# baldhat/yolov10-3D

Measured on AMD Instinct MI355X. Metric: train_images_per_sec, higher is better.
Workload: dtype bf16

## Files before the change

include/y3d.h:

```cpp
#ifndef Y3D_H
#define Y3D_H
#include <stdint.h>

#ifdef __cplusplus
extern "C" {
#endif

enum { Y3D_F32 = 0, Y3D_BF16 = 1 };
enum { Y3D_OK = 0, Y3D_ERR_INVALID = -1, Y3D_ERR_HIP = -2 };

const char* y3d_last_error(void);
int y3d_abi_version(void);
int y3d_device_info(char* name, int name_len, int* compute_units, int* lds_bytes, int* clock_khz);

int y3d_pack_weight_fwd(int dtype, const float* w_oihw, void* out, int Cout, int Cin_g, int Cin_g_pad, int kh, int kw, void* stream);
int y3d_pack_weight_dgrad(int dtype, const float* w_oihw, void* out, int Cout, int Cin_g, int groups, int kh, int kw, void* stream);
int y3d_mt_pack_weights(int dtype, const int64_t* desc, const int* chunk_tensor, const int* chunk_off, int nchunks, int chunk, void* stream);
int y3d_mt_fp8w_quantize(const int64_t* desc, const int* row_begin, int ntensors, int nrows, void* stream);
int y3d_fp8w_dequantize(const uint8_t* codes, const float* scale, float* w, int rows, int K, void* stream);
int y3d_fp8_quantize_act(const void* x, int64_t xsw, int64_t M, int C, uint8_t* q, uint8_t* s, void* stream);
int y3d_fp8_pack_weight_fwd(const uint8_t* codes, const float* scale, int rows, int Cg, uint8_t* wq, uint8_t* ws, void* stream);
int y3d_conv3x3_fp8_ok(int B, int H, int W, int Cin, int Cout, int groups);
int y3d_conv3x3_fp8_stat_rows(int B, int H, int W);
int y3d_fp8_scale_pitch(int C);
int y3d_conv3x3_fp8_fwd(const uint8_t* xq, const uint8_t* xs, int B, int H, int W, int Cin, const uint8_t* wq, const uint8_t* ws, void* y, int64_t ysw,
                        int Cout, int groups, float* stat_partials, const float* scale, const float* shift, int act, void* stream);
int y3d_fp8_quantize_grad(const void* dy, int64_t sw, const float* scale, int64_t M, int C, uint8_t* q, uint8_t* s, void* stream);
int y3d_fp8_pack_weight_dgrad(const uint8_t* codes, int Cout, int Cin, int groups, int lo, int hi, uint8_t* wq, uint8_t* ws, void* stream);
int y3d_conv3x3_fp8_dgrad_ok(int B, int H, int W, int Cin, int Cout, int groups);
int y3d_conv3x3_fp8_dgrad(const uint8_t* dyq, const uint8_t* dys, int64_t qsw, int spitch, int lo, int hi, int B, int H, int W, const uint8_t* wq, const uint8_t* ws,
                          void* dx, int64_t dxsw, int Cin, int groups, void* stream);
int y3d_conv_kpad(int dtype, int k_total);
int y3d_conv_stat_blocks(int B, int Ho, int Wo);
int y3d_conv2d_stat_rows(int dtype, int B, int H, int W, int Cin, int Cout, int groups, int kh, int kw, int stride, int pad);
enum { Y3D_OP_FWD = 0, Y3D_OP_BWD_DATA = 1, Y3D_OP_BWD_WEIGHT = 2 };
enum { Y3D_EPI_RAW = 0, Y3D_EPI_PARTIALS = 1, Y3D_EPI_AFFINE = 2, Y3D_EPI_AFFINE_RES = 3, Y3D_EPI_BIAS = 4 };
enum {
  Y3D_ROUTE_GENERIC = 0,
  Y3D_ROUTE_STREAM1X1 = 1,
  Y3D_ROUTE_SMALL = 2,
  Y3D_ROUTE_SMALL_S2 = 3,
  Y3D_ROUTE_S2_DGRAD = 4,
  Y3D_ROUTE_TILE8 = 5,
  Y3D_ROUTE_TILE16 = 6,
  Y3D_ROUTE_WIDE3_8 = 7,
  Y3D_ROUTE_WIDE3_16 = 8,
  Y3D_ROUTE_FLAT = 9,
  Y3D_ROUTE_WGRAD_SMALL = 10,
  Y3D_ROUTE_WGRAD_TILE = 11,
  Y3D_ROUTE_WGRAD_STREAM1X1 = 12
};
int y3d_conv2d_route(int dtype, int op, int epi, int B, int H, int W, int Cin, int Cout, int groups, int kh, int kw, int stride, int pad);
int y3d_conv2d_fwd(int dtype, const void* x, int64_t xsb, int64_t xsh, int64_t xsw, int B, int H, int W, int Cin,
                   const void* w_packed, const float* bias, void* y, int64_t ysw, int Ho, int Wo, int Cout, int groups,
                   int kh, int kw, int stride, int pad, float* stat_partials, void* stream);
int y3d_conv2d_fwd_affine(int dtype, const void* x, int64_t xsb, int64_t xsh, int64_t xsw, int B, int H, int W, int Cin,
                          const void* w_packed, const float* scale, const float* shift, int act, void* y, int64_t ysw, int Ho, int Wo,
                          int Cout, int groups, int kh, int kw, int stride, int pad, void* stream);
int y3d_conv2d_fwd_affine_res_ok(int dtype, int B, int H, int W, int Cin, int Cout, int groups, int kh, int kw, int stride, int pad);
int y3d_conv2d_fwd_affine_res(int dtype, const void* x, int64_t xsb, int64_t xsh, int64_t xsw, int B, int H, int W, int Cin,
                              const void* w_packed, const float* scale, const float* shift, int act, const void* res, int64_t rsw, void* y,
                              int64_t ysw, int Ho, int Wo, int Cout, int groups, int kh, int kw, int stride, int pad, void* stream);
int y3d_conv2d_bwd_data(int dtype, const void* dy, int64_t dsb, int64_t dsh, int64_t dsw, int B, int Ho, int Wo, int Cout,
                        const void* w_packed_dgrad, void* dx, int64_t xsw, int H, int W, int Cin, int groups, int kh, int kw,
                        int stride, int pad, void* stream);
int y3d_conv2d_wgrad_splits(int dtype, int B, int Ho, int Wo, int Cout, int Cin_g, int groups, int kh, int kw);
int y3d_conv2d_wgrad_plan(int dtype, int B, int H, int W, int Cin, int Cout, int groups, int kh, int kw, int stride, int pad);
int y3d_set_tile_kernels(int enable);
int y3d_set_stream1x1(int enable);
int y3d_get_stream1x1(void);
int y3d_get_tile_kernels(void);
int y3d_set_bn_wide_slabs(int enable);
int y3d_conv2d_bwd_weight(int dtype, const void* x, int64_t xsb, int64_t xsh, int64_t xsw, int B, int H, int W, int Cin,
                          int Cin_real, const void* dy, int64_t dsw, int Ho, int Wo, int Cout, int groups, int kh, int kw,
                          int stride, int pad, float* slab, int nsplit, float* grad_oihw, int accumulate, void* stream);

int y3d_dw_blocks(int64_t M);
int y3d_dw_wgrad_blocks(int64_t M);
int y3d_dw_pack_weight(const float* w_oihw, float* out_taps_c, int C, int kh, int kw, void* stream);
int y3d_dwconv2d_fwd(int dtype, const void* x, int64_t xsb, int64_t xsh, int64_t xsw, int B, int H, int W, int C,
                     const float* w_packed, void* y, int64_t ysw, int Ho, int Wo, int kh, int kw, int stride, int pad,
                     float* stat_partials, void* stream);
int y3d_dwconv2d_fwd_affine(int dtype, const void* x, int64_t xsb, int64_t xsh, int64_t xsw, int B, int H, int W, int C,
                            const float* w_packed, const float* scale, const float* shift, int act, int res_mode, const void* res, int64_t rsw,
                            void* z, int64_t zsw, int Ho, int Wo, int kh, int kw, int stride, int pad, void* stream);
int y3d_dwconv2d_bwd_data(int dtype, const void* dy, int64_t dsb, int64_t dsh, int64_t dsw, int B, int Ho, int Wo, int C,
                          const float* w_packed, void* dx, int64_t xsw, int H, int W, int kh, int kw, int stride, int pad,
                          void* stream);
int y3d_dwconv2d_bwd_weight(int dtype, const void* x, int64_t xsb, int64_t xsh, int64_t xsw, int B, int H, int W, int C,
                            const void* dy, int64_t dsw, int Ho, int Wo, int kh, int kw, int stride, int pad, float* slab,
                            float* grad_oihw, int accumulate, void* stream);

int y3d_bn_finalize(const float* partials, int nblk, int C, int64_t count, const float* gamma, const float* beta, float eps,
                    float momentum, float* running_mean, float* running_var, float* mean, float* invstd, float* scale,
                    float* shift, void* stream);
int y3d_bn_eval_scale(int C, const float* gamma, const float* beta, const float* running_mean, const float* running_var,
                      float eps, float* scale, float* shift, void* stream);
int y3d_bn_act_fwd(int dtype, const void* y, int64_t ysw, const float* scale, const float* shift, int act, int res_mode,
                   const void* res, int64_t rsw, void* z, int64_t zsw, int64_t P, int C, void* stream);
int y3d_bn_act_fwd_q(const void* y, int64_t ysw, const float* scale, const float* shift, int act, void* z, int64_t zsw, uint8_t* q, uint8_t* s,
                     int64_t P, int C, void* stream);
int y3d_bn_bwd_blocks(int64_t P, int C);
int y3d_bn_act_bwd_reduce(int dtype, const void* y, int64_t ysw, const void* dz, int64_t dsw, const void* res, int64_t rsw,
                          const float* scale, const float* shift, const float* mean, const float* invstd, int act,
                          int res_mode, float* partials, int64_t P, int C, void* stream);
int y3d_bn_bwd_finalize(const float* partials, int nblk, int C, int64_t count, float* dgamma, float* dbeta, int accumulate,
                        float* mean_g, float* mean_gx, void* stream);
int y3d_bn_act_bwd_apply(int dtype, const void* y, int64_t ysw, const void* dz, int64_t dsw, const void* res, int64_t rsw,
                         const float* scale, const float* shift, const float* mean, const float* invstd,
                         const float* mean_g, const float* mean_gx, int act, int res_mode, int train, void* dy, int64_t dysw,
                         void* dres, int64_t drsw, int64_t P, int C, void* stream);
int y3d_colsum_partials(int dtype, const void* x, int64_t xsw, float* partials, int64_t P, int C, void* stream);

int y3d_maxpool_fwd(int dtype, const void* x, int64_t xsb, int64_t xsh, int64_t xsw, void* y, int64_t ysw, uint8_t* argmax,
                    int B, int H, int W, int C, int k, void* stream);
int y3d_maxpool_bwd(int dtype, const void* dy, int64_t dsw, const uint8_t* argmax, void* dx, int64_t xsw, int B, int H, int W,
                    int C, int k, void* stream);
int y3d_upsample2x_fwd(int dtype, const void* x, int64_t xsb, int64_t xsh, int64_t xsw, void* y, int64_t ysw, int B, int H, int W,
                       int C, void* stream);
int y3d_upsample2x_bwd(int dtype, const void* dy, int64_t dsb, int64_t dsh, int64_t dsw, void* dx, int64_t xsw, int B, int H,
                       int W, int C, void* stream);
int y3d_copy2d(int dtype, const void* x, int64_t xsw, void* y, int64_t ysw, int64_t P, int C, void* stream);
int y3d_occupy_cus(int n, const int* flag, float* buf, int64_t nbuf, void* stream);
int y3d_add2d(int dtype, const void* a, int64_t asw, const void* b, int64_t bsw, void* y, int64_t ysw, int64_t P, int C, void* stream);
int y3d_nchw_to_nhwc(int dtype, const float* x_nchw, void* y_nhwc, int B, int C, int H, int W, int Cpad, void* stream);
int y3d_stem_im2col(int dtype, const float* x_nchw, void* out, int B, int H, int W, int Ho, int Wo, void* stream);
int y3d_stem_im2col_u8(int dtype, const uint8_t* x, int hwc, void* out, int B, int H, int W, int Ho, int Wo, void* stream);
int y3d_stem_conv_eval(const void* x, int in_mode, const float* wcol, const float* scale, const float* shift, int act, void* y, int64_t ysw,
                       int B, int H, int W, int Cout, void* stream);
int y3d_stem_conv_train_rows(int B, int H, int W);
int y3d_stem_conv_train(const void* x, int in_mode, const float* wcol, void* y, int64_t ysw, void* xcol, float* part, int B, int H, int W,
                        int Cout, void* stream);
int y3d_nhwc_to_nchw(int dtype, const void* x_nhwc, int64_t xsw, float* y_nchw, int B, int C, int H, int W, void* stream);
int y3d_proj_fwd(int dtype, const void* x, int64_t xsw, const float* w, const float* bias, void* y, int64_t ysw, int64_t P,
                 int Cin, int Cout, void* stream);
int y3d_proj_bwd_data(int dtype, const void* dy, int64_t dsw, const float* w, void* dx, int64_t xsw, int64_t P, int Cin, int Cout,
                      void* stream);
int y3d_proj_blocks(int64_t P);
int y3d_proj_bwd_weight(int dtype, const void* x, int64_t xsw, const void* dy, int64_t dsw, float* slab, float* bias_slab,
                        float* grad_w, float* grad_b, int accumulate, int64_t P, int Cin, int Cout, void* stream);
int y3d_slab_reduce(const float* slab, float* out, int nblk, int64_t n, int accumulate, void* stream);
int y3d_proj_group_fwd(int dtype, int nb, int cin, const void* x, int64_t xsw, const int* xoff, const float* const* w,
                       const float* const* b, const int* couts, void* y, int64_t ysw, int64_t P, void* stream);
int y3d_proj_group_bwd_data(int dtype, int nb, int cin, const void* dy, int64_t dsw, const int* xoff, const float* const* w,
                            const int* couts, void* dx, int64_t xsw, int64_t P, void* stream);
int y3d_proj_group_fwd_bn_mfma(int nb, int cin, const void* y_pre, int64_t ysw, const int* xoff, const float* const* w, const float* const* b,
                               const int* couts, const float* scale, const float* shift, int act, void* out, int64_t osw, int64_t P,
                               void* stream);
int y3d_proj_group_bwd_weight_bn_mfma_blocks(int64_t P);
int y3d_proj_group_bwd_weight_bn_mfma(int nb, int cin, const void* y_pre, int64_t ysw, const int* xoff, const void* dout, int64_t dsw,
                                      const int* couts, const float* scale, const float* shift, int act, float* slab, float* bslab,
                                      float* const* dw, float* const* db, int64_t P, void* stream);
int y3d_proj_group_bn_bwd_blocks(int64_t P);
int y3d_proj_group_bn_bwd(int mode, int nb, int cin, const void* y_pre, int64_t ysw, const int* xoff, const void* dout, int64_t dsw,
                          const float* const* w, const int* couts, const float* scale, const float* shift, const float* mean,
                          const float* invstd, const float* mean_g, const float* mean_gx, int act, float* partials, int nblk, void* dy,
                          int64_t dysw, int64_t P, int C, void* stream);
int y3d_proj_group_blocks(int64_t P);
int y3d_proj_group_fwd_bn(int dtype, int nb, int cin, const void* y_pre, int64_t xsw, const int* xoff, const float* const* w,
                          const float* const* b, const int* couts, const float* scale, const float* shift, int act, void* out,
                          int64_t ysw, int64_t P, void* stream);
int y3d_proj_group_bwd_weight_bn(int dtype, int nb, int cin, const void* y_pre, int64_t xsw, const int* xoff, const void* dy, int64_t dsw,
                                 const int* couts, const float* scale, const float* shift, int act, float* slab, float* bslab,
                                 float* const* dw, float* const* db, int64_t P, void* stream);
int y3d_proj_group_bwd_weight(int dtype, int nb, int cin, const void* x, int64_t xsw, const int* xoff, const void* dy, int64_t dsw,
                              const int* couts, float* slab, float* bslab, float* const* dw, float* const* db, int64_t P, void* stream);

int y3d_attn_fwd(int dtype, const void* qkv, int64_t qsw, void* out, int64_t osw, float* lse, int B, int N, int nh, int kd, int hd,
                 float scale, void* stream);
int y3d_attn_bwd(int dtype, const void* qkv, int64_t qsw, const void* out, int64_t osw, const void* dout, int64_t dsw,
                 const void* dv_extra, int64_t esw, const float* lse, float* delta, void* dqkv, int64_t gsw, int B, int N, int nh,
                 int kd, int hd, float scale, void* stream);

int y3d_tal3d_scratch_floats(int B, int n, int A, int topk);
int y3d_pad_targets(const float* rows, int nbox, int width, int B, int cap, float scale_x, float scale_y, float* out, int* n_used,
                    void* stream);
int y3d_tal3d_assign(int dtype, int nl, const void* const* maps, const int64_t* psw, const int* H, const int* W, const float* strides,
                     int B, int nc, const float* gt, int n, const float* calib, const float* mean_sizes, int topk, float alpha,
                     float beta, float gamma, int mode, float* scratch, uint8_t* fg_mask, int* target_gt_idx, float* target_scores, float* scal,
                     const int* n_used, void* stream);
int y3d_loss3d(int dtype, int nl, const void* const* maps, const int64_t* psw, void* const* grads, const int64_t* gsw, const int* H,
               const int* W, const float* strides, int B, int nc, const float* gt, int n, const uint8_t* fg_mask,
               const int* target_gt_idx, const float* target_scores, const float* scal, float w_loss2d, float w_cls, float w_depth,
               float w_offset3d, float w_size3d, float w_heading, float grad_scale, float* partials, float* items, void* stream);

int y3d_distill_loss(int dtype, int nl, const void* const* embs, const int64_t* psw, const int* H, const int* W, int B, int C,
                     const void* teacher, int teacher_dtype, int th, int tw, int64_t tsb, int64_t tsc, int64_t tsh, int64_t tsw,
                     const float* gt, int n, const uint8_t* fg_mask, const int* target_gt_idx, const float* scal, const uint8_t* mixed,
                     int img_w, int img_h, float T, float weight, int criterion, int no_mixup, int cap, int* counts, int* idx,
                     void* rows, float* partials, float* loss, void* stream);
int y3d_distill_scatter(int dtype, const void* rows, const int* idx, const int* nrows, const float* scale, int cap, int C, void* grad,
                        int64_t sb, int64_t sh, int64_t sw, int a0, int H, int W, void* stream);

int y3d_tal2d_assign(int dtype, int nl, const void* const* maps, const int64_t* psw, const int* H, const int* W, const float* strides,
                     int B, int nc, const float* gt, int n, int topk, float alpha, float beta, float* scratch, uint8_t* fg_mask,
                     int* target_gt_idx, float* target_scores, float* scal, const int* n_used, void* stream);
int y3d_loss2d(int dtype, int nl, const void* const* maps, const int64_t* psw, void* const* grads, const int64_t* gsw, const int* H,
               const int* W, const float* strides, int B, int nc, const float* gt, int n, const uint8_t* fg_mask,
               const int* target_gt_idx, const float* target_scores, const float* scal, float w_box, float w_cls, float w_dfl,
               float grad_scale, float* partials, float* items, void* stream);
int y3d_tal2d_scratch_floats(int B, int n, int A, int topk);
int y3d_tal2d_assign_crowded(int dtype, int nl, const void* const* maps, const int64_t* psw, const int* H, const int* W, const float* strides,
                             int B, int nc, const float* gt, int n, int topk, float alpha, float beta, float* scratch, uint8_t* fg_mask,
                             int* target_gt_idx, float* target_scores, float* scal, const int* n_used, void* stream);

int y3d_topk_cells(int dtype, const void* cls, int64_t psw, int B, int HW, int nc, int K, int* out_idx, void* stream);
int y3d_patch_gather(int dtype, const void* x, int64_t xsb, int64_t xsh, int64_t xsw, const int* idx, void* out, int B, int H, int W,
                     int C, int K, int ps, void* stream);
int y3d_head3d_scatter(int dtype, const void* cls, int64_t csw, const void* reg, int64_t rsw, const int* idx, void* map, int B, int HW,
                       int nc, int no, int K, void* stream);
int y3d_head3d_decode(int dtype, int nl, const void* const* maps, const int* H, const int* W, const float* strides, int B, int nc,
                      float* y, void* stream);
int y3d_head2d_decode(int dtype, int nl, const void* const* maps, const int* H, const int* W, const float* strides, int B, int nc,
                      float* y, void* stream);
int y3d_v10_postprocess_scratch_floats(int B, int A, int nc, int max_det);
int y3d_v10_postprocess(const float* y, int B, int C, int A, int nc, int max_det, int boxes_first, float* reg, float* scores,
                        int64_t* labels, float* scratch, void* stream);

int y3d_kitti_image_aug(const unsigned char* const* src, const unsigned char* const* src2, const int* hw, const int* flip, const double* trans_inv,
                        int B, int out_h, int out_w, int mode, void* out, void* stream);
int y3d_kde_depth_fusion(const float* predsO, int B, int K, const float* predsM, int KM, int C, float thres, float iou_thres, int nprop,
                         float* out, void* stream);
int y3d_kitti_decode(const float* preds, int B, int K, const double* calib, const double* ratio, const double* inv_trans,
                     const double* mean_size, int nc, int use_camera_dis, double threshold, double* out, unsigned char* keep, void* stream);
int y3d_kitti_encode_labels(const double* rec, const int* img_i, const double* img_f, int B, int out_w, int out_h, double min_depth,
                            double max_depth, int use_camera_dis, const double* mean_size, int n_cls, int max_objs, int64_t* cls,
                            double* bboxes, float* center_2d, float* size_2d, double* center_3d, double* size_3d, double* depth,
                            int64_t* heading_bin, double* heading_res, float* batch_idx, int* counts, double* calib, double* ratio_pad,
                            void* stream);
int y3d_kitti_plan_batch(const int64_t* img_off, const int* frame_hw, const int* rec_span, const float* P2, int N,
                         const unsigned char* arena, const double* draws_host, const double* draws, int B, const unsigned char** src,
                         const unsigned char** src2, int* hw, int* flip, double* trans_inv, int* img_i, double* img_f,
                         unsigned char* mixed, void* stream);
int y3d_json3d_encode_labels(const double* rec, const int* img_i, const double* img_f, int B, int dataset, int out_w, int out_h,
                             double min_depth, double max_depth, int use_camera_dis, const double* mean_size, int n_cls, int max_objs,
                             int64_t* cls, double* bboxes, float* center_2d, float* size_2d, double* center_3d, double* size_3d,
                             double* depth, int64_t* heading_bin, double* heading_res, float* batch_idx, int* counts, double* calib,
                             double* ratio_pad, void* stream);
int y3d_yolo2d_image_aug(const unsigned char* const* src, int n_src, const int* rec_i, const double* rec_f, const unsigned char* lut, int B,
                         int imgsz, int mode, void* out, void* stream);
int y3d_yolo2d_encode_labels(const float* rec, int n_rec, const int* lab_i, const float* lab_f, int B, int imgsz, int cap, float* cls,
                             float* bboxes, float* batch_idx, int* counts, void* stream);
int y3d_letterbox_image(const unsigned char* const* src_table, int n_src, const int* rec, int B, int H, int W, int mode, void* out,
                        void* stream);
// ... 55 lines not shown
```

yolov10-3d_amd/csrc/common.h:

```cpp
#pragma once
#include <hip/hip_runtime.h>
#include <stdint.h>

#include "../../include/y3d.h"

typedef unsigned short bf16_t;
typedef __attribute__((ext_vector_type(8))) __bf16 bf16x8_t;
typedef __attribute__((ext_vector_type(4))) float f32x4_t;
typedef __attribute__((ext_vector_type(4))) short s16x4_t;

#define Y3D_WAVE 64

__device__ __forceinline__ float bf2f(bf16_t v) { return __uint_as_float(((unsigned)v) << 16); }
__device__ __forceinline__ bf16_t f2bf(float f) {
  __bf16 b = (__bf16)f;
  return __builtin_bit_cast(unsigned short, b);
}

template <typename T> struct TT;
template <> struct TT<float> {
  static constexpr int CE = 4;
  static constexpr int BKE = 32;
  __device__ static __forceinline__ float ld(const float* p) { return *p; }
  __device__ static __forceinline__ void st(float* p, float v) { *p = v; }
  __device__ static __forceinline__ float rnd(float v) { return v; }
};
template <> struct TT<bf16_t> {
  static constexpr int CE = 8;
  static constexpr int BKE = 64;
  __device__ static __forceinline__ float ld(const bf16_t* p) { return bf2f(*p); }
  __device__ static __forceinline__ void st(bf16_t* p, float v) { *p = f2bf(v); }
  __device__ static __forceinline__ float rnd(float v) { return bf2f(f2bf(v)); }
};

template <typename T> struct Chunk;
template <> struct Chunk<float> {
  __device__ static __forceinline__ void unpack(const uint4& u, float* f) {
    f[0] = __uint_as_float(u.x); f[1] = __uint_as_float(u.y); f[2] = __uint_as_float(u.z); f[3] = __uint_as_float(u.w);
  }
  __device__ static __forceinline__ uint4 pack(const float* f) {
    return make_uint4(__float_as_uint(f[0]), __float_as_uint(f[1]), __float_as_uint(f[2]), __float_as_uint(f[3]));
  }
};
template <> struct Chunk<bf16_t> {
  __device__ static __forceinline__ void unpack(const uint4& u, float* f) {
    f[0] = __uint_as_float(u.x << 16); f[1] = __uint_as_float(u.x & 0xffff0000u);
    f[2] = __uint_as_float(u.y << 16); f[3] = __uint_as_float(u.y & 0xffff0000u);
    f[4] = __uint_as_float(u.z << 16); f[5] = __uint_as_float(u.z & 0xffff0000u);
    f[6] = __uint_as_float(u.w << 16); f[7] = __uint_as_float(u.w & 0xffff0000u);
  }
  __device__ static __forceinline__ uint4 pack(const float* f) {
    uint4 u;
    u.x = (unsigned)f2bf(f[0]) | ((unsigned)f2bf(f[1]) << 16);
    u.y = (unsigned)f2bf(f[2]) | ((unsigned)f2bf(f[3]) << 16);
    u.z = (unsigned)f2bf(f[4]) | ((unsigned)f2bf(f[5]) << 16);
    u.w = (unsigned)f2bf(f[6]) | ((unsigned)f2bf(f[7]) << 16);
    return u;
  }
};

__device__ __forceinline__ float fast_sigmoid_f(float u) { return __builtin_amdgcn_rcpf(1.f + __expf(-u)); }
__device__ __forceinline__ float silu_f(float u) { return u * fast_sigmoid_f(u); }
__device__ __forceinline__ float silu_grad_f(float u) {
  float s = fast_sigmoid_f(u);
  return s * (1.f + u * (1.f - s));
}

__device__ __forceinline__ float lane_xor8_sum(float v) {
  return v + __int_as_float(__builtin_amdgcn_update_dpp(0, __float_as_int(v), 0x128, 0xf, 0xf, false));
}
__device__ __forceinline__ float lane_xor16_sum(float v) {
  auto r = __builtin_amdgcn_permlane16_swap(__float_as_uint(v), __float_as_uint(v), false, false);
  return __uint_as_float(r[0]) + __uint_as_float(r[1]);
}
__device__ __forceinline__ float lane_xor32_sum(float v) {
  auto r = __builtin_amdgcn_permlane32_swap(__float_as_uint(v), __float_as_uint(v), false, false);
  return __uint_as_float(r[0]) + __uint_as_float(r[1]);
}

__device__ __forceinline__ float wave_xor_sum16(float v) {
  v += __int_as_float(__builtin_amdgcn_update_dpp(0, __float_as_int(v), 0xB1, 0xf, 0xf, false));
  v += __int_as_float(__builtin_amdgcn_update_dpp(0, __float_as_int(v), 0x4E, 0xf, 0xf, false));
  v += __int_as_float(__builtin_amdgcn_update_dpp(0, __float_as_int(v), 0x141, 0xf, 0xf, false));
  v += __int_as_float(__builtin_amdgcn_update_dpp(0, __float_as_int(v), 0x140, 0xf, 0xf, false));
  return v;
}

void y3d_set_error(const char* fmt, ...);
#define Y3D_CHECK(cond, ...)          \
  do {                                \
    if (!(cond)) {                    \
      y3d_set_error(__VA_ARGS__);     \
      return Y3D_ERR_INVALID;         \
    }                                 \
  } while (0)
#define Y3D_LAUNCH_CHECK()                                   \
  do {                                                       \
    hipError_t e_ = hipGetLastError();                       \
    if (e_ != hipSuccess) {                                  \
      y3d_set_error("HIP launch: %s", hipGetErrorString(e_)); \
      return Y3D_ERR_HIP;                                    \
    }                                                        \
  } while (0)

#define Y3D_HIP(call)                                                 \
  do {                                                                \
    hipError_t e_ = (call);                                           \
    if (e_ != hipSuccess) {                                           \
      y3d_set_error("%s: %s", #call, hipGetErrorString(e_));          \
      return Y3D_ERR_HIP;                                             \
    }                                                                 \
  } while (0)

static inline int cdiv(long a, long b) { return (int)((a + b - 1) / b); }
```

yolov10-3d_amd/csrc/conv_gemm.hip:

```cpp
#include "common.h"
#include "conv_frag.h"
#include <cstdlib>

namespace {

struct ConvP {
  const void* x;
  const void* w;
  const float* bias;
  const float* scale;
  const float* shift;
  int act;
  void* y;
  float* part;
  long xsb, xsh, xsw;
  long ysw;
  int B, Hg, Wg;
  int Hq, Wq;
  int Cg, Cn, G;
  int kh, kw, stride, pad;
  int Ktot, Kpad;
  int M;
  int ntx, nty;
};
// ... 329 lines not shown
  const T* __restrict__ X = (const T*)p.x;
  const T* __restrict__ D = (const T*)p.dy;

  const int mbeg = split * p.chunk_px;
  const int mend = min(p.M, mbeg + p.chunk_px);
  const int nsteps = (mend - mbeg + BPK - 1) / BPK;

  const int ccd = tid % CPD, rd0 = tid / CPD;
  const int ccx = tid % CPX, rx0 = tid / CPX;
  constexpr int RSD = 256 / CPD, RSX = 256 / CPX;
  const bool tdv = BPK * CPD >= 256 || tid < BPK * CPD, txv = BPK * CPX >= 256 || tid < BPK * CPX;
  const int kx = j0 + ccx * CE;
  const bool kx_ok = txv && kx < p.Ktot;
  int tap = 0, ci = 0, tr = 0, tq = 0;
  if (kx_ok) { tap = kx / p.Cg; ci = kx - tap * p.Cg; tr = tap / p.kw; tq = tap - tr * p.kw; }
  const int cd = i0 + ccd * CE;
  const bool cd_ok = tdv && cd < p.Cn;
  const int HW = p.Ho * p.Wo;

  uint4 rd[ND], rx[NX];
  int rb_[NX], rh_[NX], rw_[NX];
#pragma unroll
  for (int i = 0; i < NX; ++i) {
    int m = mbeg + rx0 + RSX * i;
    int b = m / HW;
    int rem = m - b * HW;
    rb_[i] = b;
    rh_[i] = rem / p.Wo;
    rw_[i] = rem - rh_[i] * p.Wo;
  }
  const T* dcol = D + (long)g * p.Cn + cd;
  const T* xcol = X + (long)g * p.Cg + ci + (long)(tr - p.pad) * p.xsh + (long)(tq - p.pad) * p.xsw;
  auto gload = [&](int st) {
#pragma unroll
    for (int i = 0; i < ND; ++i) {
      int m = mbeg + st * BPK + rd0 + RSD * i;
      uint4 vd = make_uint4(0, 0, 0, 0);
      if (m < mend && cd_ok) vd = *(const uint4*)(dcol + (long)m * p.dsw);
      rd[i] = vd;
    }
#pragma unroll
    for (int i = 0; i < NX; ++i) {
      int m = mbeg + st * BPK + rx0 + RSX * i;
      uint4 vx = make_uint4(0, 0, 0, 0);
      if (m < mend && kx_ok) {
        int hh = rh_[i] * p.stride - p.pad + tr, ww = rw_[i] * p.stride - p.pad + tq;
        if (hh >= 0 && ww >= 0 && hh < p.H && ww < p.W)
          vx = *(const uint4*)(xcol + (long)rb_[i] * p.xsb + (long)(rh_[i] * p.stride) * p.xsh + (long)(rw_[i] * p.stride) * p.xsw);
      }
      rx[i] = vx;
      rw_[i] += BPK;
      while (rw_[i] >= p.Wo) { rw_[i] -= p.Wo; ++rh_[i]; }
      while (rh_[i] >= p.Ho) { rh_[i] -= p.Ho; ++rb_[i]; }
    }
  };
  auto lstore = [&](int buf) {
    if (tdv) {
#pragma unroll
      for (int i = 0; i < ND; ++i) *(uint4*)(sD + buf * BPK * PD + (rd0 + RSD * i) * PD + ccd * 16) = rd[i];
    }
    if (txv) {
#pragma unroll
      for (int i = 0; i < NX; ++i) *(uint4*)(sX + buf * BPK * PX + (rx0 + RSX * i) * PX + ccx * 16) = rx[i];
    }
  };

  f32x4_t acc[TA][TB];
#pragma unroll
  for (int a = 0; a < TA; ++a)
#pragma unroll
    for (int b = 0; b < TB; ++b) acc[a][b] = (f32x4_t){0.f, 0.f, 0.f, 0.f};

  if (nsteps > 0) {
    gload(0);
    lstore(0);
  }
  __syncthreads();
  for (int st = 0; st < nsteps; ++st) {
    const int cur = st & 1;
    if (st + 1 < nsteps) gload(st + 1);
    const char* tD = sD + cur * BPK * PD;
    const char* tX = sX + cur * BPK * PX;
#pragma unroll
    for (int k0 = 0; k0 < BPK; k0 += TFrag<T, WD>::KSUB_PX) {
      typename TFrag<T, WD>::type fa[TA], fb[TB];
#pragma unroll
      for (int a = 0; a < TA; ++a) fa[a] = TFrag<T, WD>::load(tD, wi * (WD / 2) + a * 16, k0, lane);
#pragma unroll
      for (int b = 0; b < TB; ++b) fb[b] = TFrag<T, WX>::load(tX, wj * (WX / 2) + b * 16, k0, lane);
#pragma unroll
      for (int a = 0; a < TA; ++a)
#pragma unroll
        for (int b = 0; b < TB; ++b) acc[a][b] = TFrag<T, WD>::mma(fa[a], fb[b], acc[a][b]);
    }
    if (st + 1 < nsteps) lstore(cur ^ 1);
    __syncthreads();
  }
  float* slab = p.slab + ((long)split * p.G * p.Cn + (long)g * p.Cn) * p.Ktot;
#pragma unroll
  for (int a = 0; a < TA; ++a)
#pragma unroll
    for (int b = 0; b < TB; ++b) {
      int k = j0 + wj * (WX / 2) + b * 16 + (lane & 15);
#pragma unroll
      for (int r = 0; r < 4; ++r) {
        int co = i0 + wi * (WD / 2) + a * 16 + (lane >> 4) * 4 + r;
        if (co < p.Cn && k < p.Ktot) slab[(long)co * p.Ktot + k] = acc[a][b][r];
      }
    }
}

template <int SL>
__global__ __launch_bounds__(256) void wgrad_reduce_kernel(const float* __restrict__ slab, float* __restrict__ grad, int nsplit, int Ctot,
                                                           int taps, int Cg, int Cg_real, int accumulate) {
  constexpr int GPB = 256 / SL;
  __shared__ float4 sh[SL][GPB];
  const int e = threadIdx.x % GPB, sl = threadIdx.x / GPB;
  const long idx = ((long)blockIdx.x * GPB + e) * 4;
  const long n = (long)Ctot * taps * Cg;
  float4 s = make_float4(0.f, 0.f, 0.f, 0.f);
  if (idx < n) {
    float4 s0 = s, s1 = s, s2 = s, s3 = s;
    auto add = [](float4& a, const float4 b) { a.x += b.x; a.y += b.y; a.z += b.z; a.w += b.w; };
    int k = sl;
    for (; k + 3 * SL < nsplit; k += 4 * SL) {
      const float4 v0 = *(const float4*)(slab + (long)k * n + idx), v1 = *(const float4*)(slab + (long)(k + SL) * n + idx);
      const float4 v2 = *(const float4*)(slab + (long)(k + 2 * SL) * n + idx), v3 = *(const float4*)(slab + (long)(k + 3 * SL) * n + idx);
      add(s0, v0); add(s1, v1); add(s2, v2); add(s3, v3);
    }
    for (; k < nsplit; k += SL) add(s0, *(const float4*)(slab + (long)k * n + idx));
    s.x = (s0.x + s1.x) + (s2.x + s3.x); s.y = (s0.y + s1.y) + (s2.y + s3.y);
    s.z = (s0.z + s1.z) + (s2.z + s3.z); s.w = (s0.w + s1.w) + (s2.w + s3.w);
  }
  if (SL > 1) {
    sh[sl][e] = s;
    __syncthreads();
    if (sl != 0) return;
#pragma unroll
    for (int j = 1; j < SL; ++j) { const float4 v = sh[j][e]; s.x += v.x; s.y += v.y; s.z += v.z; s.w += v.w; }
  }
  if (idx >= n) return;
  const int ci = (int)(idx % Cg);
  const int tap = (int)((idx / Cg) % taps);
  const int co = (int)(idx / ((long)Cg * taps));
  const float v[4] = {s.x, s.y, s.z, s.w};
#pragma unroll
  for (int j = 0; j < 4; ++j) {
    if (ci + j >= Cg_real) break;
    const long o = ((long)co * Cg_real + ci + j) * taps + tap;
    grad[o] = accumulate ? grad[o] + v[j] : v[j];
  }
}

template <int SL>
__global__ __launch_bounds__(256) void wgrad_reduce_scalar_kernel(const float* __restrict__ slab, float* __restrict__ grad, int nsplit, int Ctot,
                                                           int taps, int Cg, int Cg_real, int accumulate) {
  constexpr int EPB = 256 / SL;
  __shared__ float sh[SL][EPB];
  const int e = threadIdx.x % EPB, sl = threadIdx.x / EPB;
  long idx = (long)blockIdx.x * EPB + e;
  long n = (long)Ctot * taps * Cg;
  float s = 0.f;
  if (idx < n) {
    float s0 = 0.f, s1 = 0.f, s2 = 0.f, s3 = 0.f;
    int k = sl;
    for (; k + 3 * SL < nsplit; k += 4 * SL) {
      s0 += slab[(long)k * n + idx];
      s1 += slab[(long)(k + SL) * n + idx];
      s2 += slab[(long)(k + 2 * SL) * n + idx];
      s3 += slab[(long)(k + 3 * SL) * n + idx];
    }
    for (; k < nsplit; k += SL) s0 += slab[(long)k * n + idx];
    s = (s0 + s1) + (s2 + s3);
  }
  if (SL > 1) {
    sh[sl][e] = s;
    __syncthreads();
    if (sl != 0) return;
#pragma unroll
    for (int j = 1; j < SL; ++j) s += sh[j][e];
  }
  if (idx >= n) return;
  int ci = idx % Cg;
  int tap = (idx / Cg) % taps;
  int co = idx / ((long)Cg * taps);
  if (ci >= Cg_real) return;
  long o = ((long)co * Cg_real + ci) * taps + tap;
  grad[o] = accumulate ? grad[o] + s : s;
}

inline void launch_wgrad_reduce(const float* slab, float* grad, int nsplit, int Ctot, int taps, int Cg, int Cg_real, int accumulate, hipStream_t st) {
  long n = (long)Ctot * taps * Cg;
  long ng = (n + 3) / 4;
  if (n <= 65536 && nsplit >= 64) hipLaunchKernelGGL(wgrad_reduce_kernel<16>, dim3(cdiv(ng, 16)), dim3(256), 0, st, slab, grad, nsplit, Ctot, taps, Cg, Cg_real, accumulate);
  else if (n <= 1048576 && nsplit >= 32) hipLaunchKernelGGL(wgrad_reduce_kernel<8>, dim3(cdiv(ng, 32)), dim3(256), 0, st, slab, grad, nsplit, Ctot, taps, Cg, Cg_real, accumulate);
  else if (nsplit >= 8) hipLaunchKernelGGL(wgrad_reduce_kernel<2>, dim3(cdiv(ng, 128)), dim3(256), 0, st, slab, grad, nsplit, Ctot, taps, Cg, Cg_real, accumulate);
  else hipLaunchKernelGGL(wgrad_reduce_scalar_kernel<1>, dim3(cdiv(n, 256)), dim3(256), 0, st, slab, grad, nsplit, Ctot, taps, Cg, Cg_real, accumulate);
}

template <typename T>
__global__ void pack_w_fwd_kernel(const float* __restrict__ w, T* __restrict__ out, int Cout, int Cg, int Cg_pad, int taps, int Kpad) {
  long idx = (long)blockIdx.x * blockDim.x + threadIdx.x;
  long n = (long)Cout * Kpad;
  if (idx >= n) return;
  int k = idx % Kpad;
  int co = idx / Kpad;
  float v = 0.f;
  if (k < taps * Cg_pad) {
    int tap = k / Cg_pad, ci = k - tap * Cg_pad;
    if (ci < Cg) v = w[((long)co * Cg + ci) * taps + tap];
  }
  TT<T>::st(out + idx, v);
}

template <typename T>
__global__ void pack_w_dgrad_kernel(const float* __restrict__ w, T* __restrict__ out, int G, int Cn, int Cg, int taps, int Kpad) {
  long idx = (long)blockIdx.x * blockDim.x + threadIdx.x;
  long n = (long)G * Cg * Kpad;
  if (idx >= n) return;
  int k = idx % Kpad;
  int ci = (idx / Kpad) % Cg;
  int g = idx / ((long)Kpad * Cg);
  float v = 0.f;
  if (k < taps * Cn) {
    int tap = k / Cn, co = k - tap * Cn;
    v = w[((long)(g * Cn + co) * Cg + ci) * taps + tap];
  }
  TT<T>::st(out + idx, v);
}

template <typename T>
__global__ __launch_bounds__(256) void mt_pack_w_kernel(const long* __restrict__ desc, const int* __restrict__ ctensor, const int* __restrict__ coff,
                                                        int chunk) {
  constexpr int CAP = 4096;
  __shared__ float st[CAP + 64];
  const long* d = desc + (long)ctensor[blockIdx.x] * 8;
  const float* __restrict__ w = (const float*)d[0];
  T* __restrict__ out = (T*)d[1];
  const int a = (int)d[2], b = (int)d[3], c = (int)d[4], taps = (int)d[5], Kpad = (int)d[6], mode = (int)d[7];
  const long n = mode == 0 ? (long)a * Kpad : (long)a * c * Kpad;
  const long beg = (long)coff[blockIdx.x] * chunk;
  const long end = beg + chunk < n ? beg + chunk : n;
  const int tid = threadIdx.x;
  const long rb = beg / Kpad, re = (end - 1) / Kpad;
  if (mode == 0) {
    for (long idx = beg + tid; idx < end; idx += 256) {
      const int k = (int)(idx % Kpad), co = (int)(idx / Kpad);
      float v = 0.f;
      if (k < taps * c) {
        const int tap = k / c, ci = k - tap * c;
        if (ci < b) v = w[((long)co * b + ci) * taps + tap];
      }
      TT<T>::st(out + idx, v);
    }
  } else {
    const int CB = b < 256 ? b : 256;
    int R = CAP / (taps * (CB + 1));
    if (R < 1) R = 1;
    const int P = CB + 1;
    for (long r0 = rb; r0 <= re;) {
      const int g = (int)(r0 / c), ci0 = (int)(r0 - (long)g * c);
      int nr = R;
      if (nr > c - ci0) nr = c - ci0;
      if (nr > re - r0 + 1) nr = (int)(re - r0 + 1);
      const int seg = nr * taps;
      for (int co0 = 0; co0 < b; co0 += CB) {
        const int cb = b - co0 < CB ? b - co0 : CB;
        __syncthreads();
        for (int i = tid; i < cb * seg; i += 256) {
          const int col = i / seg, j = i - col * seg;
          st[j * P + col] = w[((long)(g * b + co0 + col) * c + ci0) * taps + j];
        }
        __syncthreads();
        for (int o = tid; o < seg * cb; o += 256) {
          const int j = o / cb, col = o - j * cb;
          const int cil = j / taps, tap = j - cil * taps;
          const long idx = (r0 + cil) * Kpad + (long)tap * b + co0 + col;
          if (idx >= beg && idx < end) TT<T>::st(out + idx, st[j * P + col]);
        }
      }
      for (int o = tid; o < nr * (Kpad - taps * b); o += 256) {
        const int rl = o / (Kpad - taps * b), k = taps * b + o - rl * (Kpad - taps * b);
        const long idx = (r0 + rl) * Kpad + k;
        if (idx >= beg && idx < end) TT<T>::st(out + idx, 0.f);
      }
      r0 += nr;
    }
  }
}

template <typename T, int MODE>
int launch_conv_mode(ConvP p, hipStream_t st) {
  dim3 block(256);
  const unsigned ny = MODE == 2 ? 4 : 1;
  p.ntx = MODE == 2 ? cdiv((long)p.B * ((p.Hq + 1) / 2) * ((p.Wq + 1) / 2), 128) : cdiv(p.M, 128);
  const long t128 = (long)p.ntx * cdiv(p.Cn, 128) * ny * p.G;
  int bc = p.Cn > 64 ? 128 : (p.Cn > 32 ? 64 : 32);
  if (p.Cn % 32 == 0) {
    if (bc == 128 && t128 < 192) bc = 64;
    if (bc == 64 && (long)p.ntx * cdiv(p.Cn, 64) * ny * p.G < 192 && p.Cn > 32) bc = 32;
  }
  p.nty = cdiv(p.Cn, bc);
  if (bc == 128) {
    size_t sm = 2 * (128 + 128) * 128;
    hipLaunchKernelGGL((conv_gemm_kernel<T, 128, 128, 2, 2, MODE>), dim3(p.ntx * p.nty, ny, p.G), block, sm, st, p);
  } else if (bc == 64) {
    size_t sm = 2 * (128 + 64) * 128;
    hipLaunchKernelGGL((conv_gemm_kernel<T, 128, 64, 4, 1, MODE>), dim3(p.ntx * p.nty, ny, p.G), block, sm, st, p);
  } else {
    size_t sm = 2 * (128 + 32) * 128;
    hipLaunchKernelGGL((conv_gemm_kernel<T, 128, 32, 4, 1, MODE>), dim3(p.ntx * p.nty, ny, p.G), block, sm, st, p);
  }
  Y3D_LAUNCH_CHECK();
  return Y3D_OK;
}

template <typename T, bool DGRAD>
int launch_conv(ConvP p, hipStream_t st) {
  if (DGRAD && p.kh == 3 && p.kw == 3 && p.stride == 2 && p.pad == 1 && p.Cg % TT<T>::CE == 0) return launch_conv_mode<T, 2>(p, st);
  return launch_conv_mode<T, DGRAD ? 1 : 0>(p, st);
}

}

int y3d_conv3x3_tile_route(int dtype, int B, int H, int W, int Cg, int Cn, int G, int kh, int kw, int stride, int pad);
int y3d_conv3x3_flat_tiles(int B, int H, int W);
int y3d_conv3x3_tile_launch(int dtype, int route, const void* x, long xsb, long xsh, long xsw, int B, int H, int W, int Cg, int Cn, int G,
                            const void* w, int Ktot, void* y, long ysw, float* part, int flip, const float* scale, const float* shift, int act,
                            void* stream);

int y3d_wgrad_tile_height(int dtype, int H, int W, int Cg, int Cn, int kh, int kw, int stride, int pad);
int y3d_wgrad_tile_splits(int th, int B, int H, int W, int Cg, int Cn, int G);
int y3d_conv3x3_wgrad_tile_launch(int th, const void* x, long xsb, long xsh, long xsw, const void* dy, long dsw, int B, int H, int W, int Cg,
                                  int Cn, int G, float* slab, int nsplit, void* stream);

int y3d_conv1x1_stream_ok(int dtype, long M, int K, int N, long xsw, int G = 1);
int y3d_conv1x1_stream_launch(const void* x, long xsw, const void* w, int Kpad, const float* bias, const float* scale, const float* shift, int act,
                              void* y, long ysw, float* part, long M, int K, int N, int G, void* stream);
int y3d_wgrad1x1_stream_ok(int dtype, long M, int Cg, int Cn, long xsw, long dsw);
int y3d_wgrad1x1_stream_launch(const void* x, long xsw, const void* dy, long dsw, long M, int Cg, int Cn, float* slab, int nsplit, int chunk_px,
                               void* stream);
int y3d_conv3x3s2_dgrad_ok(int dtype, int B, int Ho, int Wo, int H, int W, int Cout, int Cin, long dsw, long xsw);
int y3d_conv3x3s2_dgrad_launch(const void* dy, long dsw, int B, int Ho, int Wo, int Cout, const void* w_packed_dgrad, int Kpad, void* dx, long xsw,
                               int H, int W, int Cin, void* stream);
int y3d_conv3x3_small_ok(int dtype, int B, int H, int W, int Cin, int Cout, int rows);
int y3d_conv3x3_small_launch(const void* x, long xsb, long xsh, long xsw, int B, int H, int W, int Cin, int Cout, const void* w, int Ktot, void* y,
                             long ysw, float* part, int rows, int flip, const float* scale, const float* shift, int act, const void* res, long rsw,
                             void* stream);
int y3d_conv3x3_small_rows(int B, int H, int W, int Cin, int Cout);
int y3d_conv3x3_small_s2_ok(int dtype, int B, int H, int W, int Cin, int Cout);
int y3d_conv3x3_small_s2_rows(int B, int H, int W, int Cin, int Cout);
int y3d_conv3x3_small_s2_launch(const void* x, long xsb, long xsh, long xsw, int B, int H, int W, int Cin, int Cout, const void* w, int Ktot, void* y,
                                long ysw, float* part, int rows, const float* scale, const float* shift, int act, void* stream);
int y3d_conv1x1_stream_rows(long M, int K, int N, int G = 1);
int y3d_wgrad3x3_small_ok(int dtype, int B, int H, int W, int Cin, int Cout);
int y3d_wgrad3x3_small_splits(int B, int H, int W);
int y3d_wgrad3x3_small_launch(const void* x, long xsb, long xsh, long xsw, const void* dy, long dsw, int B, int H, int W, int Cin, int Cout,
                              float* slab, int nsplit, void* stream);
static inline bool dense_pixels(int B, int H, int W, long sb, long sh, long sw) {
  return (H == 1 || sh == (long)W * sw) && (B == 1 || sb == (long)H * W * sw);
}

static int g_tile_kernels = 1;
extern "C" int y3d_conv2d_wgrad_splits(int dtype, int B, int Ho, int Wo, int Cout, int Cin_g, int groups, int kh, int kw);

static int conv_route(int dtype, int op, int epi, int B, int H, int W, int Ho, int Wo, int Cin, int Cout, int groups, int kh, int kw, int stride,
                      int pad, bool dense, long asw, long bsw, bool cin_full) {
  const int ce = dtype == Y3D_BF16 ? 8 : 4;
  const bool k1 = kh == 1 && kw == 1 && stride == 1 && pad == 0, k3s1 = kh == 3 && kw == 3 && stride == 1 && pad == 1,
             k3s2 = kh == 3 && kw == 3 && stride == 2 && pad == 1;
  if (op == Y3D_OP_FWD) {
    Y3D_CHECK(dtype == Y3D_BF16 || dtype == Y3D_F32, "conv2d_fwd: bad dtype %d", dtype);
    Y3D_CHECK(B > 0 && H > 0 && W > 0 && Cin > 0 && Cout > 0 && groups > 0, "conv2d_fwd: empty shape");
    Y3D_CHECK(Cin % groups == 0 && Cout % groups == 0, "conv2d_fwd: channels not divisible by groups");
    Y3D_CHECK((Cin / groups) % ce == 0, "conv2d_fwd: Cin/groups=%d must be a multiple of %d (pad the input)", Cin / groups, ce);
    Y3D_CHECK(kh * kw <= 64, "conv2d_fwd: at most 64 filter taps");
    Y3D_CHECK(epi >= Y3D_EPI_RAW && epi <= Y3D_EPI_BIAS, "conv2d_fwd: bad epilogue %d", epi);
    const int Cg = Cin / groups, Cn = Cout / groups;
    const long M = (long)B * Ho * Wo;
    const bool bias = epi == Y3D_EPI_BIAS;
    if (k1 && dense && y3d_conv1x1_stream_ok(dtype, M, Cg, Cn, asw, groups)) return Y3D_ROUTE_STREAM1X1;
    Y3D_CHECK(!(epi == Y3D_EPI_PARTIALS && k1 && y3d_conv1x1_stream_ok(dtype, M, Cg, Cn, Cin, groups)),
              "conv2d_fwd: 1x1 input view must be pixel-dense and below 4 GB for the BatchNorm partial layout of this shape");
    if (k3s1 && groups == 1 && !bias && y3d_conv3x3_small_ok(dtype, B, H, W, Cin, Cout, 1)) return Y3D_ROUTE_SMALL;
    Y3D_CHECK(epi != Y3D_EPI_AFFINE_RES, "conv2d_fwd_affine_res: no kernel with a residual epilogue takes this geometry (ask y3d_conv2d_fwd_affine_res_ok first)");
    if (k3s2 && groups == 1 && !bias && y3d_conv3x3_small_s2_ok(dtype, B, H, W, Cin, Cout)) return Y3D_ROUTE_SMALL_S2;
    if (!bias && g_tile_kernels) return y3d_conv3x3_tile_route(dtype, B, H, W, Cg, Cn, groups, kh, kw, stride, pad);
    return Y3D_ROUTE_GENERIC;
  }
  if (op == Y3D_OP_BWD_DATA) {
    Y3D_CHECK(dtype == Y3D_BF16 || dtype == Y3D_F32, "conv2d_bwd_data: bad dtype %d", dtype);
    Y3D_CHECK(groups > 0 && Cin % groups == 0 && Cout % groups == 0, "conv2d_bwd_data: channels not divisible by groups");
    Y3D_CHECK((Cout / groups) % ce == 0, "conv2d_bwd_data: Cout/groups=%d must be a multiple of %d", Cout / groups, ce);
    Y3D_CHECK(kh * kw <= 64, "conv2d_bwd_data: at most 64 filter taps");
    Y3D_CHECK(epi == 0, "conv2d_bwd_data: no epilogue variants");
    const int Cg = Cout / groups, Cn = Cin / groups;
    if (k1 && dense && y3d_conv1x1_stream_ok(dtype, (long)B * H * W, Cg, Cn, asw, groups)) return Y3D_ROUTE_STREAM1X1;
    if (k3s1 && groups == 1 && Ho == H && Wo == W && y3d_conv3x3_small_ok(dtype, B, H, W, Cout, Cin, 1)) return Y3D_ROUTE_SMALL;
    if (k3s2 && groups == 1 && dense && y3d_conv3x3s2_dgrad_ok(dtype, B, Ho, Wo, H, W, Cout, Cin, asw, bsw)) return Y3D_ROUTE_S2_DGRAD;
    if (g_tile_kernels && Ho == H && Wo == W) return y3d_conv3x3_tile_route(dtype, B, H, W, Cg, Cn, groups, kh, kw, stride, pad);
    return Y3D_ROUTE_GENERIC;
  }
  Y3D_CHECK(op == Y3D_OP_BWD_WEIGHT, "conv2d_route: bad op %d", op);
  Y3D_CHECK(dtype == Y3D_BF16 || dtype == Y3D_F32, "conv2d_bwd_weight: bad dtype %d", dtype);
  Y3D_CHECK(groups > 0 && Cin % groups == 0 && Cout % groups == 0, "conv2d_bwd_weight: channels not divisible by groups");
  Y3D_CHECK((Cin / groups) % ce == 0 && (Cout / groups) % ce == 0, "conv2d_bwd_weight: per-group channels must be multiples of %d", ce);
  Y3D_CHECK(epi == 0, "conv2d_bwd_weight: no epilogue variants");
  if (k3s1 && groups == 1 && cin_full && y3d_wgrad3x3_small_ok(dtype, B, H, W, Cin, Cout)) return Y3D_ROUTE_WGRAD_SMALL;
  if (g_tile_kernels && cin_full && y3d_wgrad_tile_height(dtype, H, W, Cin / groups, Cout / groups, kh, kw, stride, pad)) return Y3D_ROUTE_WGRAD_TILE;
  if (k1 && groups == 1 && cin_full && dense && y3d_wgrad1x1_stream_ok(dtype, (long)B * Ho * Wo, Cin, Cout, asw, bsw)) return Y3D_ROUTE_WGRAD_STREAM1X1;
  return Y3D_ROUTE_GENERIC;
}

extern "C" {

int y3d_get_tile_kernels(void) { return g_tile_kernels; }

int y3d_set_tile_kernels(int enable) {
  int old = g_tile_kernels;
  g_tile_kernels = enable ? 1 : 0;
  return old;
}

int y3d_conv_stat_blocks(int B, int Ho, int Wo) { return cdiv((long)B * Ho * Wo, 128); }

int y3d_conv2d_route(int dtype, int op, int epi, int B, int H, int W, int Cin, int Cout, int groups, int kh, int kw, int stride, int pad) {
  Y3D_CHECK(kh > 0 && kw > 0 && stride > 0 && pad >= 0, "conv2d_route: bad filter geometry");
  const int Ho = (H + 2 * pad - kh) / stride + 1, Wo = (W + 2 * pad - kw) / stride + 1;
  Y3D_CHECK(Ho > 0 && Wo > 0, "conv2d_route: empty output");
  if (op == Y3D_OP_BWD_DATA) return conv_route(dtype, op, epi, B, H, W, Ho, Wo, Cin, Cout, groups, kh, kw, stride, pad, true, Cout, Cin, true);
  return conv_route(dtype, op, epi, B, H, W, Ho, Wo, Cin, Cout, groups, kh, kw, stride, pad, true, Cin, Cout, true);
}

int y3d_conv2d_wgrad_plan(int dtype, int B, int H, int W, int Cin, int Cout, int groups, int kh, int kw, int stride, int pad) {
  int Ho = (H + 2 * pad - kh) / stride + 1, Wo = (W + 2 * pad - kw) / stride + 1;
  switch (conv_route(dtype, Y3D_OP_BWD_WEIGHT, 0, B, H, W, Ho, Wo, Cin, Cout, groups, kh, kw, stride, pad, true, Cin, Cout, true)) {
    case Y3D_ROUTE_WGRAD_SMALL: return y3d_wgrad3x3_small_splits(B, H, W);
    case Y3D_ROUTE_WGRAD_TILE:
      return y3d_wgrad_tile_splits(y3d_wgrad_tile_height(dtype, H, W, Cin / groups, Cout / groups, kh, kw, stride, pad), B, H, W, Cin / groups,
// ... 56 lines not shown
}

static int check_align(const char* what, const void* ptr, long s0, long s1, long s2, int ce) {
  Y3D_CHECK(((uintptr_t)ptr & 15) == 0, "%s: pointer not 16-byte aligned", what);
  Y3D_CHECK(s0 % ce == 0 && s1 % ce == 0 && s2 % ce == 0, "%s: strides (%ld,%ld,%ld) not multiples of %d elements", what, s0, s1, s2, ce);
  return Y3D_OK;
}

static int conv2d_fwd_impl(int dtype, const void* x, int64_t xsb, int64_t xsh, int64_t xsw, int B, int H, int W, int Cin,
                           const void* w_packed, const float* bias, const float* scale, const float* shift, int act, void* y, int64_t ysw,
                           int Ho, int Wo, int Cout, int groups, int kh, int kw, int stride, int pad, float* stat_partials, void* stream,
                           const void* res = nullptr, int64_t rsw = 0) {
  int ce = dtype == Y3D_BF16 ? 8 : 4;
  Y3D_CHECK(!(bias && stat_partials), "conv2d_fwd: bias and BN partials are mutually exclusive");
  const int epi = res ? Y3D_EPI_AFFINE_RES : scale ? Y3D_EPI_AFFINE : stat_partials ? Y3D_EPI_PARTIALS : bias ? Y3D_EPI_BIAS : Y3D_EPI_RAW;
  const int route = conv_route(dtype, Y3D_OP_FWD, epi, B, H, W, Ho, Wo, Cin, Cout, groups, kh, kw, stride, pad, dense_pixels(B, H, W, xsb, xsh, xsw),
                               xsw, 0, true);
  if (route < 0) return route;
  Y3D_CHECK(Ho == (H + 2 * pad - kh) / stride + 1 && Wo == (W + 2 * pad - kw) / stride + 1, "conv2d_fwd: output dims (%d,%d) inconsistent", Ho, Wo);
  Y3D_CHECK(ysw >= Cout, "conv2d_fwd: ysw < Cout");
  if (check_align("conv2d_fwd x", x, xsb, xsh, xsw, ce)) return Y3D_ERR_INVALID;
  Y3D_CHECK(((uintptr_t)w_packed & 15) == 0 && ((uintptr_t)y & 7) == 0, "conv2d_fwd: w/y alignment");
  Y3D_CHECK((long)B * Ho * Wo < (1L << 31), "conv2d_fwd: too many pixels");
  ConvP p;
  p.x = x; p.w = w_packed; p.bias = bias; p.scale = scale; p.shift = shift; p.act = act; p.y = y; p.part = stat_partials;
  p.xsb = xsb; p.xsh = xsh; p.xsw = xsw; p.ysw = ysw;
  p.B = B; p.Hg = H; p.Wg = W; p.Hq = Ho; p.Wq = Wo;
  p.Cg = Cin / groups; p.Cn = Cout / groups; p.G = groups;
  p.kh = kh; p.kw = kw; p.stride = stride; p.pad = pad;
  p.Ktot = kh * kw * p.Cg; p.Kpad = p.Ktot; p.M = B * Ho * Wo;
  switch (route) {
    case Y3D_ROUTE_STREAM1X1:
      return y3d_conv1x1_stream_launch(x, xsw, w_packed, p.Kpad, bias, scale, shift, act, y, ysw, stat_partials, p.M, p.Cg, p.Cn, groups, stream);
    case Y3D_ROUTE_SMALL: {
      const int rows = stat_partials ? y3d_conv3x3_small_rows(B, H, W, Cin, Cout) : 1;
      return y3d_conv3x3_small_launch(x, xsb, xsh, xsw, B, H, W, Cin, Cout, w_packed, p.Ktot, y, ysw, stat_partials, rows, 0, scale, shift, act, res, rsw, stream);
    }
    case Y3D_ROUTE_SMALL_S2: {
      const int rows = stat_partials ? y3d_conv3x3_small_s2_rows(B, H, W, Cin, Cout) : 1;
      return y3d_conv3x3_small_s2_launch(x, xsb, xsh, xsw, B, H, W, Cin, Cout, w_packed, p.Ktot, y, ysw, stat_partials, rows, scale, shift, act, stream);
    }
    case Y3D_ROUTE_GENERIC:
      if (dtype == Y3D_BF16) return launch_conv<bf16_t, false>(p, (hipStream_t)stream);
      return launch_conv<float, false>(p, (hipStream_t)stream);
    default:
      return y3d_conv3x3_tile_launch(dtype, route, x, xsb, xsh, xsw, B, H, W, p.Cg, p.Cn, groups, w_packed, p.Ktot, y, ysw, stat_partials, 0, scale,
                                     shift, act, stream);
  }
}

int y3d_conv2d_fwd(int dtype, const void* x, int64_t xsb, int64_t xsh, int64_t xsw, int B, int H, int W, int Cin,
                   const void* w_packed, const float* bias, void* y, int64_t ysw, int Ho, int Wo, int Cout, int groups,
                   int kh, int kw, int stride, int pad, float* stat_partials, void* stream) {
  return conv2d_fwd_impl(dtype, x, xsb, xsh, xsw, B, H, W, Cin, w_packed, bias, nullptr, nullptr, 0, y, ysw, Ho, Wo, Cout, groups, kh, kw,
                         stride, pad, stat_partials, stream);
}

int y3d_conv2d_fwd_affine(int dtype, const void* x, int64_t xsb, int64_t xsh, int64_t xsw, int B, int H, int W, int Cin,
                          const void* w_packed, const float* scale, const float* shift, int act, void* y, int64_t ysw, int Ho, int Wo,
                          int Cout, int groups, int kh, int kw, int stride, int pad, void* stream) {
  Y3D_CHECK(scale && shift, "conv2d_fwd_affine: scale/shift required");
  return conv2d_fwd_impl(dtype, x, xsb, xsh, xsw, B, H, W, Cin, w_packed, nullptr, scale, shift, act, y, ysw, Ho, Wo, Cout, groups, kh, kw,
                         stride, pad, nullptr, stream);
}

int y3d_conv2d_fwd_affine_res_ok(int dtype, int B, int H, int W, int Cin, int Cout, int groups, int kh, int kw, int stride, int pad) {
  return kh == 3 && kw == 3 && stride == 1 && pad == 1 && groups == 1 && y3d_conv3x3_small_ok(dtype, B, H, W, Cin, Cout, 1);
}

int y3d_conv2d_fwd_affine_res(int dtype, const void* x, int64_t xsb, int64_t xsh, int64_t xsw, int B, int H, int W, int Cin,
                              const void* w_packed, const float* scale, const float* shift, int act, const void* res, int64_t rsw, void* y,
                              int64_t ysw, int Ho, int Wo, int Cout, int groups, int kh, int kw, int stride, int pad, void* stream) {
  Y3D_CHECK(scale && shift && res, "conv2d_fwd_affine_res: scale / shift / residual required");
  Y3D_CHECK(y3d_conv2d_fwd_affine_res_ok(dtype, B, H, W, Cin, Cout, groups, kh, kw, stride, pad), "conv2d_fwd_affine_res: geometry not supported");
  return conv2d_fwd_impl(dtype, x, xsb, xsh, xsw, B, H, W, Cin, w_packed, nullptr, scale, shift, act, y, ysw, Ho, Wo, Cout, groups, kh, kw,
                         stride, pad, nullptr, stream, res, rsw);
}

int y3d_conv2d_bwd_data(int dtype, const void* dy, int64_t dsb, int64_t dsh, int64_t dsw, int B, int Ho, int Wo, int Cout,
                        const void* w_packed_dgrad, void* dx, int64_t xsw, int H, int W, int Cin, int groups, int kh, int kw,
                        int stride, int pad, void* stream) {
  int ce = dtype == Y3D_BF16 ? 8 : 4;
  const int route = conv_route(dtype, Y3D_OP_BWD_DATA, 0, B, H, W, Ho, Wo, Cin, Cout, groups, kh, kw, stride, pad,
                               dense_pixels(B, Ho, Wo, dsb, dsh, dsw), dsw, xsw, true);
  if (route < 0) return route;
  Y3D_CHECK(xsw >= Cin, "conv2d_bwd_data: xsw < Cin");
  Y3D_CHECK(stride >= 1 && dsh % stride == 0 && dsw % stride == 0, "conv2d_bwd_data: stride %d must divide the dy strides", stride);
  if (check_align("conv2d_bwd_data dy", dy, dsb, dsh, dsw, ce)) return Y3D_ERR_INVALID;
  ConvP p;
  p.x = dy; p.w = w_packed_dgrad; p.bias = nullptr; p.scale = nullptr; p.shift = nullptr; p.act = 0; p.y = dx; p.part = nullptr;
  p.xsb = dsb; p.xsh = dsh; p.xsw = dsw; p.ysw = xsw;
  p.B = B; p.Hg = Ho; p.Wg = Wo; p.Hq = H; p.Wq = W;
  p.Cg = Cout / groups; p.Cn = Cin / groups; p.G = groups;
  p.kh = kh; p.kw = kw; p.stride = stride; p.pad = pad;
  p.Ktot = kh * kw * p.Cg; p.Kpad = y3d_conv_kpad(dtype, p.Ktot); p.M = B * H * W;
  switch (route) {
    case Y3D_ROUTE_STREAM1X1:
      return y3d_conv1x1_stream_launch(dy, dsw, w_packed_dgrad, p.Kpad, nullptr, nullptr, nullptr, 0, dx, xsw, nullptr, p.M, p.Cg, p.Cn, groups, stream);
    case Y3D_ROUTE_SMALL:
      return y3d_conv3x3_small_launch(dy, dsb, dsh, dsw, B, H, W, Cout, Cin, w_packed_dgrad, p.Kpad, dx, xsw, nullptr, 1, 1, nullptr, nullptr, 0, nullptr, 0, stream);
    case Y3D_ROUTE_S2_DGRAD:
      return y3d_conv3x3s2_dgrad_launch(dy, dsw, B, Ho, Wo, Cout, w_packed_dgrad, p.Kpad, dx, xsw, H, W, Cin, stream);
    case Y3D_ROUTE_GENERIC:
      if (dtype == Y3D_BF16) return launch_conv<bf16_t, true>(p, (hipStream_t)stream);
      return launch_conv<float, true>(p, (hipStream_t)stream);
    default:
      return y3d_conv3x3_tile_launch(dtype, route, dy, dsb, dsh, dsw, B, H, W, p.Cg, p.Cn, groups, w_packed_dgrad, p.Kpad, dx, xsw, nullptr, 1, nullptr,
                                     nullptr, 0, stream);
  }
}

static inline int wgrad_tile_w(int n) { return n <= 32 ? 32 : (n <= 64 ? 64 : 128); }

int y3d_conv2d_wgrad_splits(int dtype, int B, int Ho, int Wo, int Cout, int Cin_g, int groups, int kh, int kw) {
  int bpk = dtype == Y3D_BF16 ? 64 : 32;
  long M = (long)B * Ho * Wo;
  long tiles = (long)cdiv(kh * kw * Cin_g, wgrad_tile_w(kh * kw * Cin_g)) * cdiv(Cout / groups, wgrad_tile_w(Cout / groups)) * groups;
  long slab = (long)Cout * kh * kw * Cin_g * 4;
  long want = cdiv(slab <= (1 << 20) ? 1024 : 512, tiles);
  long maxs = cdiv(M, 4 * bpk);
  if (want > maxs) want = maxs;
  long cap = (32L << 20) / slab;
  if (cap < 128) cap = 128;
  if (want > cap) want = cap;
  if (want > 1024) want = 1024;
  if (want < 1) want = 1;
  return (int)want;
}

int y3d_conv2d_bwd_weight(int dtype, const void* x, int64_t xsb, int64_t xsh, int64_t xsw, int B, int H, int W, int Cin,
                          int Cin_real, const void* dy, int64_t dsw, int Ho, int Wo, int Cout, int groups, int kh, int kw,
                          int stride, int pad, float* slab, int nsplit, float* grad_oihw, int accumulate, void* stream) {
  int ce = dtype == Y3D_BF16 ? 8 : 4;
  int bpk = dtype == Y3D_BF16 ? 64 : 32;
  const int route = conv_route(dtype, Y3D_OP_BWD_WEIGHT, 0, B, H, W, Ho, Wo, Cin, Cout, groups, kh, kw, stride, pad, dense_pixels(B, H, W, xsb, xsh, xsw),
                               xsw, dsw, Cin_real == Cin);
  if (route < 0) return route;
  Y3D_CHECK(nsplit >= 1, "conv2d_bwd_weight: nsplit");
  Y3D_CHECK(Cin_real <= Cin && (Cin_real == Cin || groups == 1), "conv2d_bwd_weight: Cin_real");
  if (check_align("conv2d_bwd_weight x", x, xsb, xsh, xsw, ce)) return Y3D_ERR_INVALID;
  Y3D_CHECK(((uintptr_t)dy & 15) == 0 && dsw % ce == 0, "conv2d_bwd_weight: dy alignment");
  WgradP p;
  p.x = x; p.dy = dy; p.slab = slab;
  p.xsb = xsb; p.xsh = xsh; p.xsw = xsw; p.dsw = dsw;
  p.B = B; p.H = H; p.W = W; p.Ho = Ho; p.Wo = Wo;
  p.Cg = Cin / groups; p.Cn = Cout / groups; p.G = groups;
  p.kh = kh; p.kw = kw; p.stride = stride; p.pad = pad;
  p.Ktot = kh * kw * p.Cg; p.M = B * Ho * Wo; p.nsplit = nsplit;
  p.chunk_px = cdiv(cdiv(p.M, nsplit), bpk) * bpk;
  hipStream_t st = (hipStream_t)stream;
  if (route == Y3D_ROUTE_WGRAD_SMALL) {
    int rc = y3d_wgrad3x3_small_launch(x, xsb, xsh, xsw, dy, dsw, B, H, W, Cin, Cout, slab, nsplit, stream);
    if (rc) return rc;
    launch_wgrad_reduce(slab, grad_oihw, nsplit, Cout, 9, Cin, Cin, accumulate, st);
    Y3D_LAUNCH_CHECK();
    return Y3D_OK;
  }
  if (route == Y3D_ROUTE_WGRAD_TILE) {
    const int th = y3d_wgrad_tile_height(dtype, H, W, p.Cg, p.Cn, kh, kw, stride, pad);
    Y3D_CHECK(nsplit == y3d_wgrad_tile_splits(th, B, H, W, p.Cg, p.Cn, groups), "conv2d_bwd_weight: nsplit must come from y3d_conv2d_wgrad_plan");
    int rc = y3d_conv3x3_wgrad_tile_launch(th, x, xsb, xsh, xsw, dy, dsw, B, H, W, p.Cg, p.Cn, groups, slab, nsplit, stream);
    if (rc) return rc;
    launch_wgrad_reduce(slab, grad_oihw, nsplit, Cout, kh * kw, p.Cg, p.Cg, accumulate, st);
    Y3D_LAUNCH_CHECK();
    return Y3D_OK;
  }
  if (route == Y3D_ROUTE_WGRAD_STREAM1X1) {
    int rc = y3d_wgrad1x1_stream_launch(x, xsw, dy, dsw, p.M, Cin, Cout, slab, nsplit, p.chunk_px, stream);
    if (rc) return rc;
    launch_wgrad_reduce(slab, grad_oihw, nsplit, Cout, 1, Cin, Cin, accumulate, st);
    Y3D_LAUNCH_CHECK();
    return Y3D_OK;
  }
  const int wd = wgrad_tile_w(p.Cn), wx = wgrad_tile_w(p.Ktot);
  dim3 grid(cdiv(p.Ktot, wx), cdiv(p.Cn, wd), groups * nsplit);
#define Y3D_WGRAD(T, WD, WX)                                                                                         \
  hipLaunchKernelGGL((conv_wgrad_kernel<T, WD, WX>), grid, dim3(256),                                                  \
                     2 * TT<T>::BKE * (size_t)(TFrag<T, WD>::PITCH + TFrag<T, WX>::PITCH), st, p)
#define Y3D_WGRAD_T(T)                                                                                               \
  do {                                                                                                               \
    if (wd == 128) { if (wx == 128) Y3D_WGRAD(T, 128, 128); else if (wx == 64) Y3D_WGRAD(T, 128, 64); else Y3D_WGRAD(T, 128, 32); } \
    else if (wd == 64) { if (wx == 128) Y3D_WGRAD(T, 64, 128); else if (wx == 64) Y3D_WGRAD(T, 64, 64); else Y3D_WGRAD(T, 64, 32); } \
    else { if (wx == 128) Y3D_WGRAD(T, 32, 128); else if (wx == 64) Y3D_WGRAD(T, 32, 64); else Y3D_WGRAD(T, 32, 32); }    \
  } while (0)
  if (dtype == Y3D_BF16) Y3D_WGRAD_T(bf16_t); else Y3D_WGRAD_T(float);
#undef Y3D_WGRAD_T
#undef Y3D_WGRAD
  Y3D_LAUNCH_CHECK();
  int cg_real = groups == 1 ? Cin_real : p.Cg;
  launch_wgrad_reduce(slab, grad_oihw, nsplit, Cout, kh * kw, p.Cg, cg_real, accumulate, st);
  Y3D_LAUNCH_CHECK();
  return Y3D_OK;
}

int y3d_mt_pack_weights(int dtype, const int64_t* desc, const int* chunk_tensor, const int* chunk_off, int nchunks, int chunk, void* stream) {
  Y3D_CHECK(dtype == Y3D_BF16 || dtype == Y3D_F32, "mt_pack_weights: bad dtype");
  Y3D_CHECK(nchunks >= 1 && chunk >= 256, "mt_pack_weights: empty chunk table");
  hipStream_t st = (hipStream_t)stream;
  if (dtype == Y3D_BF16) hipLaunchKernelGGL(mt_pack_w_kernel<bf16_t>, dim3(nchunks), dim3(256), 0, st, (const long*)desc, chunk_tensor, chunk_off, chunk);
  else hipLaunchKernelGGL(mt_pack_w_kernel<float>, dim3(nchunks), dim3(256), 0, st, (const long*)desc, chunk_tensor, chunk_off, chunk);
  Y3D_LAUNCH_CHECK();
  return Y3D_OK;
}

}
```

yolov10-3d_amd/csrc/dwconv.hip:

```cpp
#include "common.h"

namespace {

template <int CE>
__device__ __forceinline__ void pk_fma(float* acc, const float* a, const float* b) {
  typedef float f32x2_t __attribute__((ext_vector_type(2)));
#pragma unroll
  for (int j = 0; j < CE; j += 2) {
    const f32x2_t c2 = {acc[j], acc[j + 1]}, a2 = {a[j], a[j + 1]}, b2 = {b[j], b[j + 1]};
    const f32x2_t o2 = __builtin_elementwise_fma(a2, b2, c2);
    acc[j] = o2[0];
    acc[j + 1] = o2[1];
  }
}

struct DwP {
  const void* x;
  const float* w;
  void* y;
  float* part;
  long xsb, xsh, xsw, ysw;
  int B, Hg, Wg, Hq, Wq, C, kh, kw, stride, pad;
  long M;
  int px_per_block;
// ... 156 lines not shown
__global__ __launch_bounds__(256) void dwconv_wgrad_kernel(DwWP p) {
  constexpr int CE = TT<T>::CE;
  constexpr int CT = 64 / CE;
  constexpr int PT = 256 / CT;
  constexpr int RP = 1;
  constexpr int KW = K > 0 ? K : 8;
  __shared__ float sh[4][RP * KW * 64];
  const int ct = threadIdx.x % CT, pt = threadIdx.x / CT;
  const int kh = K > 0 ? K : p.kh, kw = K > 0 ? K : p.kw;
  const int L = blockIdx.x, jx = L >> 3;
  const int row = jx % kh, tile = (jx / kh) * 8 + (L & 7);
  if (tile >= p.nblk * p.nslab) return;
  const int bx = tile % p.nblk;
  const int cs = (tile / p.nblk) * 64;
  const int c = cs + ct * CE;
  const int taps = kh * kw;
  const T* __restrict__ X = (const T*)p.x;
  const T* __restrict__ D = (const T*)p.dy;
  const long pbeg = (long)bx * p.px_per_block;
  const long pend = pbeg + p.px_per_block < p.M ? pbeg + p.px_per_block : p.M;
  const int HWo = p.Ho * p.Wo;
  {
    const int r0 = row * RP;
    float acc[RP][KW][CE];
#pragma unroll
    for (int r = 0; r < RP; ++r)
#pragma unroll
      for (int q = 0; q < KW; ++q)
#pragma unroll
        for (int j = 0; j < CE; ++j) acc[r][q][j] = 0.f;
    if (c < p.C) {
      long m = pbeg + pt;
      int b = (int)(m / HWo);
      int rem = (int)(m - (long)b * HWo);
      int ho = rem / p.Wo, wo = rem - ho * p.Wo;
      auto one = [&](const uint4& dv, int bb, int hh0, int ww0) {
        float d[CE];
        Chunk<T>::unpack(dv, d);
        const T* xb = X + (long)bb * p.xsb + c;
        uint4 raw[RP][KW];
#pragma unroll
        for (int r = 0; r < RP; ++r) {
          const int hh = hh0 + r0 + r;
          const bool okh = r0 + r < kh && hh >= 0 && hh < p.H;
#pragma unroll
          for (int q = 0; q < KW; ++q) {
            const int ww = ww0 + q;
            const bool ok = okh && q < kw && ww >= 0 && ww < p.W;
            raw[r][q] = ok ? *(const uint4*)(xb + (long)hh * p.xsh + (long)ww * p.xsw) : make_uint4(0, 0, 0, 0);
          }
        }
#pragma unroll
        for (int r = 0; r < RP; ++r)
#pragma unroll
          for (int q = 0; q < KW; ++q) {
            float v[CE];
            Chunk<T>::unpack(raw[r][q], v);
            pk_fma<CE>(acc[r][q], d, v);
          }
      };
      auto advance = [&]() {
        wo += PT;
        while (wo >= p.Wo) { wo -= p.Wo; ++ho; }
        while (ho >= p.Ho) { ho -= p.Ho; ++b; }
      };
      for (; m + PT < pend; m += 2 * PT) {
        const uint4 d0 = *(const uint4*)(D + m * p.dsw + c), d1 = *(const uint4*)(D + (m + PT) * p.dsw + c);
        const int b0 = b, h0 = ho * p.stride - p.pad, w0 = wo * p.stride - p.pad;
        advance();
        const int b1 = b, h1 = ho * p.stride - p.pad, w1 = wo * p.stride - p.pad;
        advance();
        one(d0, b0, h0, w0);
        one(d1, b1, h1, w1);
      }
      if (m < pend) one(*(const uint4*)(D + m * p.dsw + c), b, ho * p.stride - p.pad, wo * p.stride - p.pad);
    }
    const int lane = threadIdx.x & 63, wave = threadIdx.x >> 6;
#pragma unroll
    for (int r = 0; r < RP; ++r)
#pragma unroll
      for (int q = 0; q < KW; ++q)
#pragma unroll
        for (int j = 0; j < CE; ++j) {
          float v = acc[r][q][j];
          if (CT == 8) v = lane_xor8_sum(v);
          v = lane_xor32_sum(lane_xor16_sum(v));
          if (lane < CT) sh[wave][(r * KW + q) * 64 + ct * CE + j] = v;
        }
    __syncthreads();
    for (int i = threadIdx.x; i < RP * KW * 64; i += 256) {
      const int t = i >> 6, cc = i & 63;
      const int r = t / KW, q = t - r * KW;
      if (r0 + r < kh && q < kw && cs + cc < p.C)
        p.slab[((long)bx * taps + (r0 + r) * kw + q) * p.C + cs + cc] = sh[0][i] + sh[1][i] + sh[2][i] + sh[3][i];
    }
  }
}

__global__ __launch_bounds__(256) void dw_wgrad_reduce_kernel(const float* __restrict__ slab, float* __restrict__ grad, int nblk, int taps, int C,
                                                              int accumulate) {
  __shared__ float sh[8][32];
  const int e = threadIdx.x & 31, sl = threadIdx.x >> 5;
  const int idx = blockIdx.x * 32 + e;
  const int n = taps * C;
  float s = 0.f;
  if (idx < n)
    for (int b = sl; b < nblk; b += 8) s += slab[(long)b * n + idx];
  sh[sl][e] = s;
  __syncthreads();
  if (sl != 0 || idx >= n) return;
#pragma unroll
  for (int j = 1; j < 8; ++j) s += sh[j][e];
  const int c = idx % C, t = idx / C;
  const long o = (long)c * taps + t;
  grad[o] = accumulate ? grad[o] + s : s;
}

__global__ void dw_pack_kernel(const float* __restrict__ w, float* __restrict__ out, int C, int taps) {
  int idx = blockIdx.x * blockDim.x + threadIdx.x;
  if (idx >= taps * C) return;
  int c = idx % C, t = idx / C;
  out[idx] = w[(long)c * taps + t];
}

}

extern "C" {

int y3d_dw_blocks(int64_t M) {
  long n = (M + 63) / 64;
  return (int)(n < 1 ? 1 : (n > 2048 ? 2048 : n));
}

int y3d_dw_wgrad_blocks(int64_t M) {
  long n = (M + 127) / 128;
  return (int)(n < 1 ? 1 : (n > 1024 ? 1024 : n));
}

int y3d_dw_pack_weight(const float* w_oihw, float* out, int C, int kh, int kw, void* stream) {
  hipLaunchKernelGGL(dw_pack_kernel, dim3(cdiv((long)C * kh * kw, 256)), dim3(256), 0, (hipStream_t)stream, w_oihw, out, C, kh * kw);
  Y3D_LAUNCH_CHECK();
  return Y3D_OK;
}

#define DW_LAUNCH_K(T, D, K) hipLaunchKernelGGL((dwconv_kernel<T, D, K>), grid, dim3(256), sm, st, p)
#define DW_LAUNCH_A(T, K) hipLaunchKernelGGL((dwconv_kernel<T, false, K, true>), grid, dim3(256), sm, st, p)
#define DW_LAUNCH(T)                                                                                             \
  do {                                                                                                           \
    const int kk = (p.kh == p.kw && (p.kh == 3 || p.kh == 7)) ? p.kh : 0;                                        \
    if (!dgrad && p.scale) { if (kk == 3) DW_LAUNCH_A(T, 3); else if (kk == 7) DW_LAUNCH_A(T, 7); else DW_LAUNCH_A(T, 0); }           \
    else if (dgrad) { if (kk == 3) DW_LAUNCH_K(T, true, 3); else if (kk == 7) DW_LAUNCH_K(T, true, 7); else DW_LAUNCH_K(T, true, 0); }     \
    else { if (kk == 3) DW_LAUNCH_K(T, false, 3); else if (kk == 7) DW_LAUNCH_K(T, false, 7); else DW_LAUNCH_K(T, false, 0); }        \
  } while (0)

static int dw_launch(int dtype, bool dgrad, const DwP& p, hipStream_t st) {
  Y3D_CHECK(p.M < (1L << 31), "dwconv: more than 2^31 pixels");
  int ce = dtype == Y3D_BF16 ? 8 : 4;
  int pt = 256 / (64 / ce);
  size_t sm = (size_t)(p.kh * p.kw * 64 + pt * 64 * 2) * sizeof(float);
  dim3 grid(y3d_dw_blocks(p.M), cdiv(p.C, 64));
  if (dtype == Y3D_BF16) {
    DW_LAUNCH(bf16_t);
  } else {
    DW_LAUNCH(float);
  }
  Y3D_LAUNCH_CHECK();
  return Y3D_OK;
}

int y3d_dwconv2d_fwd(int dtype, const void* x, int64_t xsb, int64_t xsh, int64_t xsw, int B, int H, int W, int C,
                     const float* w_packed, void* y, int64_t ysw, int Ho, int Wo, int kh, int kw, int stride, int pad,
                     float* stat_partials, void* stream) {
  int ce = dtype == Y3D_BF16 ? 8 : 4;
  Y3D_CHECK(dtype == Y3D_BF16 || dtype == Y3D_F32, "dwconv2d_fwd: bad dtype");
  Y3D_CHECK(C % ce == 0, "dwconv2d_fwd: C=%d not a multiple of %d", C, ce);
  Y3D_CHECK(Ho == (H + 2 * pad - kh) / stride + 1 && Wo == (W + 2 * pad - kw) / stride + 1, "dwconv2d_fwd: output dims");
  Y3D_CHECK((((uintptr_t)x | (uintptr_t)y) & 15) == 0 && xsb % ce == 0 && xsh % ce == 0 && xsw % ce == 0 && ysw % ce == 0, "dwconv2d_fwd: alignment");
  DwP p;
  p.x = x; p.w = w_packed; p.y = y; p.part = stat_partials;
  p.scale = nullptr; p.shift = nullptr; p.res = nullptr; p.rsw = 0; p.act = 0; p.res_mode = 0;
  p.xsb = xsb; p.xsh = xsh; p.xsw = xsw; p.ysw = ysw;
  p.B = B; p.Hg = H; p.Wg = W; p.Hq = Ho; p.Wq = Wo; p.C = C; p.kh = kh; p.kw = kw; p.stride = stride; p.pad = pad;
  p.M = (long)B * Ho * Wo;
  int nblk = y3d_dw_blocks(p.M);
  p.px_per_block = (int)((p.M + nblk - 1) / nblk);
  return dw_launch(dtype, false, p, (hipStream_t)stream);
}

int y3d_dwconv2d_fwd_affine(int dtype, const void* x, int64_t xsb, int64_t xsh, int64_t xsw, int B, int H, int W, int C,
                            const float* w_packed, const float* scale, const float* shift, int act, int res_mode, const void* res, int64_t rsw,
                            void* z, int64_t zsw, int Ho, int Wo, int kh, int kw, int stride, int pad, void* stream) {
  int ce = dtype == Y3D_BF16 ? 8 : 4;
  Y3D_CHECK(dtype == Y3D_BF16 || dtype == Y3D_F32, "dwconv2d_fwd_affine: bad dtype");
  Y3D_CHECK(C % ce == 0, "dwconv2d_fwd_affine: C=%d not a multiple of %d", C, ce);
  Y3D_CHECK(Ho == (H + 2 * pad - kh) / stride + 1 && Wo == (W + 2 * pad - kw) / stride + 1, "dwconv2d_fwd_affine: output dims");
  Y3D_CHECK((((uintptr_t)x | (uintptr_t)z) & 15) == 0 && xsb % ce == 0 && xsh % ce == 0 && xsw % ce == 0 && zsw % ce == 0, "dwconv2d_fwd_affine: alignment");
  Y3D_CHECK(scale && shift && res_mode >= 0 && res_mode <= 2, "dwconv2d_fwd_affine: scale / shift missing or bad residual mode");
  Y3D_CHECK(res_mode == 0 || (res && (((uintptr_t)res) & 15) == 0 && rsw % ce == 0), "dwconv2d_fwd_affine: residual missing or misaligned");
  DwP p;
  p.x = x; p.w = w_packed; p.y = z; p.part = nullptr;
  p.scale = scale; p.shift = shift; p.res = res; p.rsw = rsw; p.act = act; p.res_mode = res_mode;
  p.xsb = xsb; p.xsh = xsh; p.xsw = xsw; p.ysw = zsw;
  p.B = B; p.Hg = H; p.Wg = W; p.Hq = Ho; p.Wq = Wo; p.C = C; p.kh = kh; p.kw = kw; p.stride = stride; p.pad = pad;
  p.M = (long)B * Ho * Wo;
  int nblk = y3d_dw_blocks(p.M);
  p.px_per_block = (int)((p.M + nblk - 1) / nblk);
  return dw_launch(dtype, false, p, (hipStream_t)stream);
}

int y3d_dwconv2d_bwd_data(int dtype, const void* dy, int64_t dsb, int64_t dsh, int64_t dsw, int B, int Ho, int Wo, int C,
                          const float* w_packed, void* dx, int64_t xsw, int H, int W, int kh, int kw, int stride, int pad,
                          void* stream) {
  int ce = dtype == Y3D_BF16 ? 8 : 4;
  Y3D_CHECK(dtype == Y3D_BF16 || dtype == Y3D_F32, "dwconv2d_bwd_data: bad dtype");
  Y3D_CHECK(C % ce == 0, "dwconv2d_bwd_data: C=%d not a multiple of %d", C, ce);
  Y3D_CHECK((((uintptr_t)dy | (uintptr_t)dx) & 15) == 0 && dsb % ce == 0 && dsh % ce == 0 && dsw % ce == 0 && xsw % ce == 0, "dwconv2d_bwd_data: alignment");
  DwP p;
  p.x = dy; p.w = w_packed; p.y = dx; p.part = nullptr;
  p.scale = nullptr; p.shift = nullptr; p.res = nullptr; p.rsw = 0; p.act = 0; p.res_mode = 0;
  p.xsb = dsb; p.xsh = dsh; p.xsw = dsw; p.ysw = xsw;
  p.B = B; p.Hg = Ho; p.Wg = Wo; p.Hq = H; p.Wq = W; p.C = C; p.kh = kh; p.kw = kw; p.stride = stride; p.pad = pad;
  p.M = (long)B * H * W;
  int nblk = y3d_dw_blocks(p.M);
  p.px_per_block = (int)((p.M + nblk - 1) / nblk);
  return dw_launch(dtype, true, p, (hipStream_t)stream);
}

int y3d_dwconv2d_bwd_weight(int dtype, const void* x, int64_t xsb, int64_t xsh, int64_t xsw, int B, int H, int W, int C,
                            const void* dy, int64_t dsw, int Ho, int Wo, int kh, int kw, int stride, int pad, float* slab,
                            float* grad_oihw, int accumulate, void* stream) {
  int ce = dtype == Y3D_BF16 ? 8 : 4;
  Y3D_CHECK(dtype == Y3D_BF16 || dtype == Y3D_F32, "dwconv2d_bwd_weight: bad dtype");
  Y3D_CHECK(C % ce == 0, "dwconv2d_bwd_weight: C=%d not a multiple of %d", C, ce);
  Y3D_CHECK((((uintptr_t)x | (uintptr_t)dy) & 15) == 0 && xsb % ce == 0 && xsh % ce == 0 && xsw % ce == 0 && dsw % ce == 0, "dwconv2d_bwd_weight: alignment");
  DwWP p;
  p.x = x; p.dy = dy; p.slab = slab;
  p.xsb = xsb; p.xsh = xsh; p.xsw = xsw; p.dsw = dsw;
  p.B = B; p.H = H; p.W = W; p.Ho = Ho; p.Wo = Wo; p.C = C; p.kh = kh; p.kw = kw; p.stride = stride; p.pad = pad;
  p.M = (long)B * Ho * Wo;
  int nblk = y3d_dw_wgrad_blocks(p.M);
  p.px_per_block = (int)((p.M + nblk - 1) / nblk);
  p.nblk = nblk; p.nslab = cdiv(C, 64);
  dim3 grid(cdiv(nblk * p.nslab, 8) * 8 * kh);
  hipStream_t st = (hipStream_t)stream;
  Y3D_CHECK(kw <= 8 || (kh == kw && (kh == 3 || kh == 7)), "dwconv2d_bwd_weight: kernels wider than 8 taps are not supported");
#define Y3D_DWW(T)                                                                                                          \
  do {                                                                                                                      \
    if (kh == 3 && kw == 3) hipLaunchKernelGGL((dwconv_wgrad_kernel<T, 3>), grid, dim3(256), 0, st, p);                      \
    else if (kh == 7 && kw == 7) hipLaunchKernelGGL((dwconv_wgrad_kernel<T, 7>), grid, dim3(256), 0, st, p);                 \
    else hipLaunchKernelGGL((dwconv_wgrad_kernel<T, 0>), grid, dim3(256), 0, st, p);                                         \
  } while (0)
  if (dtype == Y3D_BF16) Y3D_DWW(bf16_t); else Y3D_DWW(float);
#undef Y3D_DWW
  Y3D_LAUNCH_CHECK();
  hipLaunchKernelGGL(dw_wgrad_reduce_kernel, dim3(cdiv((long)C * kh * kw, 32)), dim3(256), 0, st, slab, grad_oihw, nblk, kh * kw, C, accumulate);
  Y3D_LAUNCH_CHECK();
  return Y3D_OK;
}

}
```

yolov10-3d_amd/csrc/proj_bn_mfma.hip:

```cpp
#include "common.h"

namespace {

constexpr int PB_MAXB = 16;

struct PBP {
  const bf16_t* y;
  const bf16_t* dout;
  bf16_t* dy;
  float* part;
  const float* w[PB_MAXB];
  int xoff[PB_MAXB], ooff[PB_MAXB], cout[PB_MAXB];
  const float *scale, *shift, *mean, *invstd, *mg, *mgx;
  long ysw, dsw, dysw, P;
  int cin, C, act, px_per_block;
};

template <int MODE, int NT>
__global__ __launch_bounds__(256) void projg_bn_bwd_kernel(PBP p) {
  constexpr int CIN = NT * 16, LDW = CIN + 4;
  constexpr int CH = CIN / 8;
  constexpr int PPP = 64 / CH;
  constexpr int NPASS = 16 / PPP;
  static_assert(NPASS >= 1 && 64 % CH == 0 && 16 % PPP == 0, "cin must be 32, 64 or 128");
// ... 130 lines not shown
  const int c0 = p.xoff[br] + cc * 8;
  float sc[8], sf[8];
#pragma unroll
  for (int j = 0; j < 8; ++j) { sc[j] = p.scale[c0 + j]; sf[j] = p.shift[c0 + j]; }
  const long pbeg = (long)blockIdx.x * p.px_per_block;
  const long pend = pbeg + p.px_per_block < p.P ? pbeg + p.px_per_block : p.P;
  bf16_t* op = p.out + p.ooff[br];
  const bool two = cout > 16;
  for (long pb = pbeg; pb < pend; pb += 64) {
    const long p0 = pb + wave * 16;
    uint4 yv[NPASS];
#pragma unroll
    for (int s = 0; s < NPASS; ++s) {
      const long px = p0 + s * PPP + pr;
      yv[s] = px < pend ? *(const uint4*)(p.y + px * p.ysw + c0) : make_uint4(0, 0, 0, 0);
    }
#pragma unroll
    for (int s = 0; s < NPASS; ++s) {
      float v[8];
      Chunk<bf16_t>::unpack(yv[s], v);
#pragma unroll
      for (int j = 0; j < 8; ++j) {
        const float u = v[j] * sc[j] + sf[j];
        v[j] = p.act ? silu_f(u) : u;
      }
      *(uint4*)(tile + (s * PPP + pr) * LDB + cc * 16) = Chunk<bf16_t>::pack(v);
    }
    __syncthreads();
    f32x4_t acc0 = {0.f, 0.f, 0.f, 0.f}, acc1 = {0.f, 0.f, 0.f, 0.f};
#pragma unroll
    for (int ks = 0; ks < KS; ++ks) {
      const bf16x8_t a = __builtin_bit_cast(bf16x8_t, *(const uint4*)(tile + lp * LDB + (ks * 4 + q) * 16));
      acc0 = __builtin_amdgcn_mfma_f32_16x16x32_bf16(a, wf[0][ks], acc0, 0, 0, 0);
      if (two) acc1 = __builtin_amdgcn_mfma_f32_16x16x32_bf16(a, wf[1][ks], acc1, 0, 0, 0);
    }
#pragma unroll
    for (int r = 0; r < 4; ++r) {
      const long px = p0 + 4 * q + r;
      if (px < pend) {
        if (lp < cout) op[px * p.osw + lp] = f2bf(acc0[r] + bias[0]);
        if (two && 16 + lp < cout) op[px * p.osw + 16 + lp] = f2bf(acc1[r] + bias[1]);
      }
    }
    __syncthreads();
  }
}

struct PWP {
  const bf16_t* y;
  const bf16_t* dout;
  float* slab;
  float* bslab;
  float* dw[PB_MAXB];
  float* db[PB_MAXB];
  int xoff[PB_MAXB], ooff[PB_MAXB], cout[PB_MAXB];
  const float *scale, *shift;
  long ysw, dsw, P;
  int act, px_per_block, ctot;
};

template <int NT>
__global__ __launch_bounds__(256) void projg_bwd_weight_bn_mfma_kernel(PWP p) {
  constexpr int CIN = NT * 16;
  constexpr int LDB = CIN * 2 + 32;
  constexpr int CH = CIN / 8, PPP = 64 / CH, NPASS = 32 / PPP;
  extern __shared__ __attribute__((aligned(16))) float psm[];
  const int tid = threadIdx.x, lane = tid & 63, wave = tid >> 6;
  const int g = lane >> 4, lp = lane & 15;
  const int br = blockIdx.y, cout = p.cout[br];
  const bool two = cout > 16;
  char* tile = (char*)psm + wave * 32 * LDB;
  const int cc = lane % CH, pr = lane / CH;
  const int c0 = p.xoff[br] + cc * 8;
  float sc[8], sf[8];
#pragma unroll
  for (int j = 0; j < 8; ++j) { sc[j] = p.scale[c0 + j]; sf[j] = p.shift[c0 + j]; }
  f32x4_t acc[2][NT];
#pragma unroll
  for (int n = 0; n < 2; ++n)
#pragma unroll
    for (int t = 0; t < NT; ++t) acc[n][t] = (f32x4_t){0.f, 0.f, 0.f, 0.f};
  float bsum[2] = {0.f, 0.f};
  const long pbeg = (long)blockIdx.x * p.px_per_block;
  const long pend = pbeg + p.px_per_block < p.P ? pbeg + p.px_per_block : p.P;
  const bf16_t* dop = p.dout + p.ooff[br];
  const int trow = 4 * g + (lp >> 2), tcol = (lp & 3) * 4;
  for (long pb = pbeg; pb < pend; pb += 128) {
    const long p0 = pb + wave * 32;
    uint4 yv[NPASS];
#pragma unroll
    for (int s = 0; s < NPASS; ++s) {
      const long px = p0 + s * PPP + pr;
      yv[s] = px < pend ? *(const uint4*)(p.y + px * p.ysw + c0) : make_uint4(0, 0, 0, 0);
    }
    bf16x8_t a[2];
#pragma unroll
    for (int n = 0; n < 2; ++n)
#pragma unroll
      for (int j = 0; j < 8; ++j) {
        const long px = p0 + 16 * (j >> 2) + 4 * g + (j & 3);
        const int o = 16 * n + lp;
        unsigned short raw = 0;
        if ((n == 0 || two) && o < cout && px < pend) raw = dop[px * p.dsw + o];
        a[n][j] = __builtin_bit_cast(__bf16, raw);
        bsum[n] += bf2f(raw);
      }
#pragma unroll
    for (int s = 0; s < NPASS; ++s) {
      float v[8];
      Chunk<bf16_t>::unpack(yv[s], v);
#pragma unroll
      for (int j = 0; j < 8; ++j) {
        const float u = v[j] * sc[j] + sf[j];
        v[j] = p.act ? silu_f(u) : u;
      }
      *(uint4*)(tile + (s * PPP + pr) * LDB + cc * 16) = Chunk<bf16_t>::pack(v);
    }
    __syncthreads();
#pragma unroll
    for (int t = 0; t < NT; ++t) {
      const char* a0 = tile + trow * LDB + (t * 16 + tcol) * 2;
      const s16x4_t lo = __builtin_amdgcn_ds_read_tr16_b64_v4i16((s16x4_t __attribute__((address_space(3)))*)(a0));
      const s16x4_t hi = __builtin_amdgcn_ds_read_tr16_b64_v4i16((s16x4_t __attribute__((address_space(3)))*)(a0 + 16 * LDB));
      typedef __attribute__((ext_vector_type(8))) short s16x8_t;
      const bf16x8_t b = __builtin_bit_cast(bf16x8_t, (s16x8_t)__builtin_shufflevector(lo, hi, 0, 1, 2, 3, 4, 5, 6, 7));
      acc[0][t] = __builtin_amdgcn_mfma_f32_16x16x32_bf16(a[0], b, acc[0][t], 0, 0, 0);
      if (two) acc[1][t] = __builtin_amdgcn_mfma_f32_16x16x32_bf16(a[1], b, acc[1][t], 0, 0, 0);
    }
    __syncthreads();
  }
  float* red = psm;
  const int NO = two ? 2 : 1;
  for (int n = 0; n < NO; ++n)
#pragma unroll
    for (int t = 0; t < NT; ++t)
#pragma unroll
      for (int r = 0; r < 4; ++r) red[(wave * 32 + 16 * n + 4 * g + r) * CIN + t * 16 + lp] = (n == 0 ? acc[0][t][r] : acc[1][t][r]);
  __shared__ float bred[4][32];
#pragma unroll
  for (int n = 0; n < 2; ++n) {
    float v = bsum[n];
    v = lane_xor32_sum(lane_xor16_sum(v));
    if (g == 0) bred[wave][16 * n + lp] = v;
  }
  __syncthreads();
  for (int i = tid; i < cout * CIN; i += 256) {
    const int o = i / CIN, ch = i - o * CIN;
    p.slab[((long)blockIdx.x * p.ctot + p.ooff[br] + o) * CIN + ch] =
        red[(0 * 32 + o) * CIN + ch] + red[(1 * 32 + o) * CIN + ch] + red[(2 * 32 + o) * CIN + ch] + red[(3 * 32 + o) * CIN + ch];
  }
  if (tid < cout) p.bslab[(long)blockIdx.x * p.ctot + p.ooff[br] + tid] = bred[0][tid] + bred[1][tid] + bred[2][tid] + bred[3][tid];
}

__global__ void projg_wslab_reduce_kernel(PWP p, int nblk, int cin) {
  const int br = blockIdx.y, cout = p.cout[br];
  const int idx = blockIdx.x * blockDim.x + threadIdx.x;
  if (idx < cout * cin) {
    float s = 0.f;
    for (int b = 0; b < nblk; ++b) s += p.slab[((long)b * p.ctot + p.ooff[br]) * cin + idx];
    p.dw[br][idx] = s;
  }
  if (idx < cout) {
    float s = 0.f;
    for (int b = 0; b < nblk; ++b) s += p.bslab[(long)b * p.ctot + p.ooff[br] + idx];
    p.db[br][idx] = s;
  }
}

}

extern "C" {

int y3d_proj_group_bwd_weight_bn_mfma_blocks(int64_t P) {
  long n = (P + 1023) / 1024;
  return (int)(n < 1 ? 1 : (n > 64 ? 64 : n));
}

int y3d_proj_group_bwd_weight_bn_mfma(int nb, int cin, const void* y_pre, int64_t ysw, const int* xoff, const void* dout, int64_t dsw,
                                      const int* couts, const float* scale, const float* shift, int act, float* slab, float* bslab,
                                      float* const* dw, float* const* db, int64_t P, void* stream) {
  Y3D_CHECK(nb >= 1 && nb <= PB_MAXB && (cin == 64 || cin == 128), "proj_group_bwd_weight_bn_mfma: 1..16 branches of 64 or 128 channels");
  Y3D_CHECK(y_pre && dout && scale && shift && slab && bslab && dw && db && P >= 1 && ysw % 8 == 0 && ((uintptr_t)y_pre & 15) == 0,
            "proj_group_bwd_weight_bn_mfma: null / misaligned argument");
  PWP p;
  p.y = (const bf16_t*)y_pre; p.dout = (const bf16_t*)dout; p.slab = slab; p.bslab = bslab;
  int off = 0;
  for (int i = 0; i < nb; ++i) {
    Y3D_CHECK(couts[i] >= 1 && couts[i] <= 32 && xoff[i] % 8 == 0, "proj_group_bwd_weight_bn_mfma: cout in 1..32, channel slices 16-byte aligned");
    p.dw[i] = dw[i]; p.db[i] = db[i]; p.xoff[i] = xoff[i]; p.ooff[i] = off; p.cout[i] = couts[i];
    off += couts[i];
  }
  Y3D_CHECK(dsw >= off, "proj_group_bwd_weight_bn_mfma: dout pixel stride smaller than the projected channels");
  p.scale = scale; p.shift = shift; p.ysw = ysw; p.dsw = dsw; p.P = P; p.act = act; p.ctot = off;
  const int nrun = y3d_proj_group_bwd_weight_bn_mfma_blocks(P);
  p.px_per_block = (int)(((P + nrun - 1) / nrun + 127) / 128 * 128);
  hipStream_t st = (hipStream_t)stream;
  const size_t sm = (size_t)4 * 32 * cin * sizeof(float);
  static bool attr = false;
  if (!attr) {
    (void)hipFuncSetAttribute((const void*)projg_bwd_weight_bn_mfma_kernel<8>, hipFuncAttributeMaxDynamicSharedMemorySize, 4 * 32 * 128 * 4);
    (void)hipFuncSetAttribute((const void*)projg_bwd_weight_bn_mfma_kernel<4>, hipFuncAttributeMaxDynamicSharedMemorySize, 4 * 32 * 64 * 4);
    attr = true;
  }
  if (cin == 128) hipLaunchKernelGGL((projg_bwd_weight_bn_mfma_kernel<8>), dim3(nrun, nb), dim3(256), sm, st, p);
  else hipLaunchKernelGGL((projg_bwd_weight_bn_mfma_kernel<4>), dim3(nrun, nb), dim3(256), sm, st, p);
  hipLaunchKernelGGL(projg_wslab_reduce_kernel, dim3((32 * cin + 255) / 256, nb), dim3(256), 0, st, p, nrun, cin);
  Y3D_LAUNCH_CHECK();
  return Y3D_OK;
}

int y3d_proj_group_fwd_bn_mfma(int nb, int cin, const void* y_pre, int64_t ysw, const int* xoff, const float* const* w, const float* const* b,
                               const int* couts, const float* scale, const float* shift, int act, void* out, int64_t osw, int64_t P,
                               void* stream) {
  Y3D_CHECK(nb >= 1 && nb <= PB_MAXB && (cin == 64 || cin == 128), "proj_group_fwd_bn_mfma: 1..16 branches of 64 or 128 channels");
  Y3D_CHECK(y_pre && out && w && b && scale && shift && P >= 1 && ysw % 8 == 0 && ((uintptr_t)y_pre & 15) == 0, "proj_group_fwd_bn_mfma: null / misaligned argument");
  PFP p;
  p.y = (const bf16_t*)y_pre; p.out = (bf16_t*)out;
  int off = 0;
  for (int i = 0; i < nb; ++i) {
    Y3D_CHECK(couts[i] >= 1 && couts[i] <= 32 && xoff[i] % 8 == 0, "proj_group_fwd_bn_mfma: cout in 1..32, channel slices 16-byte aligned");
    p.w[i] = w[i]; p.b[i] = b[i]; p.xoff[i] = xoff[i]; p.ooff[i] = off; p.cout[i] = couts[i];
    off += couts[i];
  }
  Y3D_CHECK(osw >= off, "proj_group_fwd_bn_mfma: output pixel stride smaller than the projected channels");
  p.scale = scale; p.shift = shift; p.ysw = ysw; p.osw = osw; p.P = P; p.act = act;
  long nrun = (P + 63) / 64;
  if (nrun > 128) nrun = 128;
  p.px_per_block = (int)(((P + nrun - 1) / nrun + 63) / 64 * 64);
  dim3 grid((unsigned)nrun, nb);
  hipStream_t st = (hipStream_t)stream;
  if (cin == 128) hipLaunchKernelGGL((projg_fwd_bn_mfma_kernel<8>), grid, dim3(256), (size_t)4 * 16 * (128 * 2 + 16), st, p);
  else hipLaunchKernelGGL((projg_fwd_bn_mfma_kernel<4>), grid, dim3(256), (size_t)4 * 16 * (64 * 2 + 16), st, p);
  Y3D_LAUNCH_CHECK();
  return Y3D_OK;
}

int y3d_proj_group_bn_bwd_blocks(int64_t P) {
  long n = (P + 63) / 64;
  return (int)(n < 1 ? 1 : (n > 128 ? 128 : n));
}

int y3d_proj_group_bn_bwd(int mode, int nb, int cin, const void* y_pre, int64_t ysw, const int* xoff, const void* dout, int64_t dsw,
                          const float* const* w, const int* couts, const float* scale, const float* shift, const float* mean,
                          const float* invstd, const float* mean_g, const float* mean_gx, int act, float* partials, int nblk, void* dy,
                          int64_t dysw, int64_t P, int C, void* stream) {
  Y3D_CHECK(mode == 0 || mode == 1, "proj_group_bn_bwd: mode 0 (reduce) or 1 (apply)");
  Y3D_CHECK(nb >= 1 && nb <= PB_MAXB && (cin == 64 || cin == 128), "proj_group_bn_bwd: 1..16 branches of 64 or 128 channels");
  Y3D_CHECK(y_pre && dout && scale && shift && mean && invstd && P >= 1, "proj_group_bn_bwd: null argument");
  Y3D_CHECK(mode == 0 ? (partials != nullptr && nblk == y3d_proj_group_bn_bwd_blocks(P)) : (dy && mean_g && mean_gx && dysw >= cin),
            "proj_group_bn_bwd: partials / nblk (reduce) or dy / mean_g / mean_gx (apply) missing");
  Y3D_CHECK(ysw % 8 == 0 && ((uintptr_t)y_pre & 15) == 0 && (mode == 0 || (dysw % 8 == 0 && ((uintptr_t)dy & 15) == 0)), "proj_group_bn_bwd: 16-byte alignment");
  PBP p;
  p.y = (const bf16_t*)y_pre; p.dout = (const bf16_t*)dout; p.dy = (bf16_t*)dy; p.part = partials;
  int off = 0;
  for (int i = 0; i < nb; ++i) {
    Y3D_CHECK(couts[i] >= 1 && couts[i] <= 32 && xoff[i] % 8 == 0 && xoff[i] + cin <= C, "proj_group_bn_bwd: cout in 1..32, channel slices 16-byte aligned inside C");
    p.w[i] = w[i]; p.xoff[i] = xoff[i]; p.ooff[i] = off; p.cout[i] = couts[i];
    off += couts[i];
  }
  Y3D_CHECK(dsw >= off, "proj_group_bn_bwd: dout pixel stride smaller than the projected channels");
  p.scale = scale; p.shift = shift; p.mean = mean; p.invstd = invstd; p.mg = mean_g; p.mgx = mean_gx;
  p.ysw = ysw; p.dsw = dsw; p.dysw = dysw; p.P = P; p.cin = cin; p.C = C; p.act = act;
  const int nrun = y3d_proj_group_bn_bwd_blocks(P);
  p.px_per_block = (int)(((P + nrun - 1) / nrun + 63) / 64 * 64);
  dim3 grid(nrun, nb);
  hipStream_t st = (hipStream_t)stream;
  const size_t sm128 = (size_t)4 * 16 * (128 + 4) * sizeof(float), sm64 = (size_t)4 * 16 * (64 + 4) * sizeof(float);
  if (cin == 128) {
    if (mode == 0) hipLaunchKernelGGL((projg_bn_bwd_kernel<0, 8>), grid, dim3(256), sm128, st, p);
    else hipLaunchKernelGGL((projg_bn_bwd_kernel<1, 8>), grid, dim3(256), sm128, st, p);
  } else {
    if (mode == 0) hipLaunchKernelGGL((projg_bn_bwd_kernel<0, 4>), grid, dim3(256), sm64, st, p);
    else hipLaunchKernelGGL((projg_bn_bwd_kernel<1, 4>), grid, dim3(256), sm64, st, p);
  }
  Y3D_LAUNCH_CHECK();
  return Y3D_OK;
}

}
```

yolov10-3d_amd/ops.py:

```python
from __future__ import annotations

import os
from collections import namedtuple

import torch

from ._lib import BF16, F32, Y3DError, lib

_COMPUTE_DTYPE = torch.bfloat16


def set_compute_dtype(dt: torch.dtype):
    global _COMPUTE_DTYPE
    if dt not in (torch.bfloat16, torch.float32):
        raise ValueError("compute dtype must be torch.bfloat16 or torch.float32")
    _COMPUTE_DTYPE = dt


def compute_dtype() -> torch.dtype:
    return _COMPUTE_DTYPE


def code(dt: torch.dtype) -> int:
    if dt == torch.bfloat16:
# ... 76 lines not shown
    _CONCAT_BASE[buf.data_ptr()] = (C, buf)
    return buf


_CONCAT_BASE = {}


_GRAD_SLOT = {}


def grad_slot(x):
    ent = _GRAD_SLOT.get((x.data_ptr(), x.shape[1]))
    if ent is None:
        return None
    holder, off = ent
    if holder["shape"] != (x.shape[0], x.shape[2], x.shape[3]) or holder["dtype"] != x.dtype:
        return None
    return holder, off, x.shape[1]


def grad_slot_tensor(slot):
    holder, off, w = slot
    if holder["buf"] is None:
        B, H, W = holder["shape"]
        holder["buf"] = nhwc_empty(B, holder["C"], H, W, holder["dtype"], holder["device"])
    return holder["buf"][:, off:off + w]


def reset_placement():
    global _PLACE, _PLACE_FINAL
    _PLACE = None
    _PLACE_FINAL = None
    _CONCAT_BASE.clear()
    _GRAD_SLOT.clear()
    _FP8_ACT.clear()


def out_tensor(B, C, H, W, dtype, device):
    global _PLACE
    if _PLACE is not None:
        buf, off = _PLACE
        if (buf.dtype == dtype and buf.shape[0] == B and buf.shape[2] == H and buf.shape[3] == W and off + C <= buf.shape[1]
                and off % ce(dtype) == 0 and C % ce(dtype) == 0 and buf.device == device):
            _PLACE = None
            return buf[:, off:off + C]
    return nhwc_empty(B, C, H, W, dtype, device)


def is_nhwc(x: torch.Tensor) -> bool:
    return x.dim() == 4 and (x.stride(1) == 1 or x.shape[1] == 1)


def px_dense(x: torch.Tensor) -> bool:
    B, C, H, W = x.shape
    sw = x.stride(3)
    return is_nhwc(x) and sw >= C and (H == 1 or x.stride(2) == W * sw) and (B == 1 or x.stride(0) == H * W * sw)


def to_nhwc(x: torch.Tensor, dtype=None, dense=False) -> torch.Tensor:
    dtype = dtype or _COMPUTE_DTYPE
    c = ce(dtype)
    ok = (x.dtype == dtype and is_nhwc(x) and x.data_ptr() % 16 == 0 and x.stride(0) % c == 0 and x.stride(2) % c == 0
          and x.stride(3) % c == 0 and (not dense or px_dense(x)))
    if ok:
        return x
    B, C, H, W = x.shape
    out = nhwc_empty(B, C, H, W, dtype, x.device)
    out.copy_(x)
    return out


def s3(x):
    return x.stride(0), x.stride(2), x.stride(3)


def _f32(n, device):
    return torch.empty(n, dtype=torch.float32, device=device)


class KernelTimer:

    def __init__(self, want):
        self.want = want
        self.pending = []

    def bracket(self, key, fn):
        if not self.want(key):
            return fn()
        a, b = torch.cuda.Event(enable_timing=True), torch.cuda.Event(enable_timing=True)
        a.record()
        r = fn()
        b.record()
        self.pending.append((key, a, b))
        return r

    def results(self):
        torch.cuda.synchronize()
        out = {}
        for key, a, b in self.pending:
            out.setdefault(key, []).append(a.elapsed_time(b))
        return out


TIMER = None

PARAM_EPOCH = 0


def bump_param_epoch():
    global PARAM_EPOCH
    PARAM_EPOCH += 1


WEIGHT_EPOCH = 0


def bump_weight_epoch():
    global WEIGHT_EPOCH
    WEIGHT_EPOCH += 1
    bump_param_epoch()


class _WeightRegistry:

    KEEP = 4

    def __init__(self):
        self.entries, self.epoch, self.tables = {}, None, None
        self.captured_tables = []

    def _hold_tables(self):
        if torch.cuda.is_current_stream_capturing() and not any(t is self.tables for t in self.captured_tables):
            self.captured_tables.append(self.tables)

    def _revisit(self, e, now, ver, refresh_all):
        e["seen"] = WEIGHT_EPOCH
        capturing = torch.cuda.is_current_stream_capturing()
        if capturing:
            e["pinned"] = True
        if self.epoch != now:
            self.epoch = now
            stale = [] if capturing else [k for k, v in self.entries.items() if WEIGHT_EPOCH - v["seen"] > self.KEEP and not v.get("pinned")]
            for k in stale:
                del self.entries[k]
            for v in refresh_all():
                v["ver"] = None
        changed = e["ver"] is not None and e["ver"] != ver
        e["ver"] = ver
        return changed


class _PackRegistry(_WeightRegistry):

    CHUNK = 16384

    def __init__(self, mode):
        super().__init__()
        self.mode = mode

    def _pack_one(self, e):
        L, st = lib(), stream()
        a, b, c, taps, kpad, dt = e["geo"]
        k = int(round(taps ** 0.5))
        if self.mode == 0:
            L.pack_weight_fwd(dt, e["src"], e["dst"].data_ptr(), a, b, c, k, k, st)
        else:
            L.pack_weight_dgrad(dt, e["src"], e["dst"].data_ptr(), a * b, c, a, k, k, st)

    def _pack_all(self, dt):
        ents = [e for e in self.entries.values() if e["geo"][5] == dt]
        if not ents:
            return ents
        dev = ents[0]["dst"].device
        key = tuple(id(e) for e in ents)
        if self.tables is None or self.tables[0] != (key, dt):
            desc, ct, co = [], [], []
            for t, e in enumerate(ents):
                a, b, c, taps, kpad, _ = e["geo"]
                n = a * kpad if self.mode == 0 else a * c * kpad
                desc += [e["src"], e["dst"].data_ptr(), a, b, c, taps, kpad, self.mode]
                for j in range((n + self.CHUNK - 1) // self.CHUNK):
                    ct.append(t)
                    co.append(j)
            self.tables = ((key, dt), torch.tensor(desc, dtype=torch.int64, device=dev), torch.tensor(ct, dtype=torch.int32, device=dev),
                           torch.tensor(co, dtype=torch.int32, device=dev), len(ct))
        _, desc, ct, co, n = self.tables
        self._hold_tables()
        lib().mt_pack_weights(dt, desc.data_ptr(), ct.data_ptr(), co.data_ptr(), n, self.CHUNK, stream())
        return ents

    def lookup(self, w32, src_ptr, geo, dtype, ver=None):
        key = (src_ptr, geo)
        ver = w32._version if ver is None else ver
        e = self.entries.get(key)
        if e is None:
            a, b, c, taps, kpad, dt = geo
            n = a * kpad if self.mode == 0 else a * c * kpad
            e = {"src": src_ptr, "geo": geo, "dst": torch.empty(n, dtype=dtype, device=w32.device), "ver": ver, "seen": WEIGHT_EPOCH,
                 "keep": w32}
            self.entries[key] = e
            self._pack_one(e)
        elif self._revisit(e, (WEIGHT_EPOCH, geo[5]), ver, lambda: self._pack_all(geo[5])):
            self._pack_one(e)
        return e["dst"]


class _QuantRegistry(_WeightRegistry):

    def _run(self, ents):
        dev = ents[0]["weff"].device
        key = tuple(id(e) for e in ents)
        if self.tables is None or self.tables[0] != key:
            desc, rb, r = [], [], 0
            for e in ents:
                rows, K = e["shape"]
                desc += [e["src"], e["weff"].data_ptr(), e["codes"].data_ptr(), e["scale"].data_ptr(), rows, K]
                rb.append(r)
                r += rows
            self.tables = (key, torch.tensor(desc, dtype=torch.int64, device=dev), torch.tensor(rb, dtype=torch.int32, device=dev), len(ents), r)
        _, desc, rb, nt, nrows = self.tables
        self._hold_tables()
        lib().mt_fp8w_quantize(desc.data_ptr(), rb.data_ptr(), nt, nrows, stream())
        return ents

    def _run_one(self, e):
        tb, self.tables = self.tables, None
        self._run([e])
        self.tables = tb

    def lookup(self, w32, ver=None):
        ver = w32._version if ver is None else ver
        rows, K = w32.shape[0], w32[0].numel()
        key = (w32.data_ptr(), rows, K)
        e = self.entries.get(key)
        if e is None:
            dev = w32.device
            e = {"src": w32.data_ptr(), "shape": (rows, K), "keep": w32, "weff": torch.empty(w32.shape, dtype=torch.float32, device=dev),
                 "codes": torch.empty((rows, K), dtype=torch.uint8, device=dev), "scale": torch.empty(rows, dtype=torch.float32, device=dev),
                 "ver": ver, "count": 0, "seen": WEIGHT_EPOCH}
            self.entries[key] = e
            self._run_one(e)
        elif self._revisit(e, WEIGHT_EPOCH, ver, lambda: self._run(list(self.entries.values()))):
            e["count"] += 1
            self._run_one(e)
        self.last = e
        return e["weff"], (WEIGHT_EPOCH, e["count"])


PACK_FWD, PACK_DGRAD, QUANT = _PackRegistry(0), _PackRegistry(1), _QuantRegistry()
WEIGHT_QUANT = None


def set_weight_quant(mode):
    global WEIGHT_QUANT
    if mode not in (None, "fp8"):
        raise ValueError("weight quantisation mode must be None or 'fp8'")
    WEIGHT_QUANT = mode
    if mode is None:
        set_fp8_dgrad(False)
    bump_param_epoch()


def weight_quant():
    return WEIGHT_QUANT


FP8_CONV = False
FP8_DGRAD = False
_FP8_WANT = False
_FP8_ACT = {}


def set_fp8_conv(on: bool):
    global FP8_CONV
    if on and WEIGHT_QUANT != "fp8":
        raise ValueError('set_fp8_conv(True) needs set_weight_quant("fp8"): the kernel multiplies the fp8w quantiser\'s codes')
    FP8_CONV = bool(on)
    if not on:
        set_fp8_dgrad(False)
    bump_param_epoch()


def fp8_conv():
    return FP8_CONV


def set_fp8_dgrad(on: bool):
    global FP8_DGRAD
    if on and not FP8_CONV:
        raise ValueError("set_fp8_dgrad(True) needs set_fp8_conv(True): the data gradient follows the layers whose forward runs in fp8")
    FP8_DGRAD = bool(on)


def fp8_dgrad():
    return FP8_DGRAD


class want_fp8_copy:

    def __enter__(self):
        global _FP8_WANT
        self.prev, _FP8_WANT = _FP8_WANT, FP8_CONV
        return self

    def __exit__(self, *a):
        global _FP8_WANT
        _FP8_WANT = self.prev


def fp8_input(xin):
    B, C, H, W = xin.shape
    ent = _FP8_ACT.pop(xin.data_ptr(), None)
    if ent is not None and ent[2] == (B, C, H, W):
        return ent[0], ent[1]
    if not px_dense(xin):
        xin = to_nhwc(xin, torch.bfloat16, dense=True).contiguous(memory_format=torch.channels_last)
    q = torch.empty(B, H, W, C, dtype=torch.uint8, device=xin.device)
    s = torch.empty(B, H, W, lib().fp8_scale_pitch(C), dtype=torch.uint8, device=xin.device)
    lib().fp8_quantize_act(xin.data_ptr(), xin.stride(3), B * H * W, C, q.data_ptr(), s.data_ptr(), stream())
    return q, s


def fp8_weight(ent, Cg):
    tok = (WEIGHT_EPOCH, ent["count"])
    hit = ent.get("wq")
    if hit is None or hit[0] != tok:
        rows = ent["shape"][0]
        dev = ent["codes"].device
        wq = hit[1] if hit is not None else torch.empty(rows, 9, Cg, dtype=torch.uint8, device=dev)
        ws = hit[2] if hit is not None else torch.empty(rows, dtype=torch.uint8, device=dev)
        lib().fp8_pack_weight_fwd(ent["codes"].data_ptr(), ent["scale"].data_ptr(), rows, Cg, wq.data_ptr(), ws.data_ptr(), stream())
        hit = ent["wq"] = (tok, wq, ws)
    return hit[1], hit[2]


def fp8_weight_dgrad(ent, Cin, g, lo, hi):
    tok = (WEIGHT_EPOCH, ent["count"])
    cache = ent.setdefault("wqd", {})
    hit = cache.get((g, lo, hi))
    if hit is None or hit[0] != tok:
        Cout = ent["shape"][0]
        dev = ent["codes"].device
        wq = hit[1] if hit is not None else torch.empty(g, Cin // g, 9, (hi - lo) // g, dtype=torch.uint8, device=dev)
        ws = hit[2] if hit is not None else torch.empty(Cin, dtype=torch.uint8, device=dev)
        lib().fp8_pack_weight_dgrad(ent["codes"].data_ptr(), Cout, Cin, g, lo, hi, wq.data_ptr(), ws.data_ptr(), stream())
        hit = cache[(g, lo, hi)] = (tok, wq, ws)
    return hit[1], hit[2]


PROJ_BN_MFMA = True
STEM_FUSED = True
PACK_CACHE = True
DW_EVAL_FUSED = True


def conv_bn_act_eval(x, w, gamma, beta, rm, rv, k, s, p, g, act, eps, cache=None, ver=None):
    z, _, _ = _cba_forward(x, w, gamma, beta, rm, rv, k, s, p, g, act, None, 0, False, eps, 0.0, cache, ver=ver)
    return z


_IDENT = {}


def _identity_bn(C, device):
    ident = _IDENT.get((C, device))
    if ident is None:
        ident = _IDENT[(C, device)] = (torch.ones(C, dtype=torch.float32, device=device), torch.zeros(C, dtype=torch.float32, device=device))
    return ident


def conv_bias_act_eval(x, w, bias, k, s, p, g, act, res, res_mode, cache):
    _require_gpu(x)
    ones, zeros = _identity_bn(w.shape[0], w.device)
    with torch.no_grad():
        z, _, _ = _cba_forward(x, _w32(w), ones, bias.detach().float(), zeros, ones, k, s, p, g, act, res, res_mode, False, 0.0, 0.0, cache)
    return z


def _cache_put(cache, key, value):
    for old in [q for q in cache if q[1] != PARAM_EPOCH]:
        del cache[old]
    cache[key] = value


def _eval_consts(cache, kind, w32, g32, b32, rm, rv, ver, dtype, k, g, Cin_g, Cg_pad, Cout, eps):
    L, st, dev = lib(), stream(), w32.device
    vkey = ver[1] if ver is not None else (w32._version, g32._version, b32._version, rm._version, rv._version)
    key = (kind, PARAM_EPOCH, w32.data_ptr(), g32.data_ptr(), rm.data_ptr(), vkey, dtype, k, g, Cg_pad, Cout, float(eps))
    hit = cache.get(key) if cache is not None else None
    if hit is None:
        if kind == "dw":
            wp = _f32(k * k * Cout, dev)
            L.dw_pack_weight(w32.data_ptr(), wp.data_ptr(), Cout, k, k, st)
        else:
            wp = torch.empty(Cout * k * k * Cg_pad, dtype=dtype, device=dev)
            L.pack_weight_fwd(code(dtype), w32.data_ptr(), wp.data_ptr(), Cout, Cin_g, Cg_pad, k, k, st)
        ss = _f32(2 * Cout, dev).view(2, Cout)
        L.bn_eval_scale(Cout, g32.data_ptr(), b32.data_ptr(), rm.data_ptr(), rv.data_ptr(), eps, ss[0].data_ptr(), ss[1].data_ptr(), st)
        hit = (wp, ss, w32)
        if cache is not None:
            _cache_put(cache, key, hit)
    return hit[0], hit[1]


def _timed(key, launch):
    if TIMER is not None:
        TIMER.bracket(key, launch)
    else:
        launch()


ConvPlan = namedtuple("ConvPlan", "B Cin Cin_k H W Cout Ho Wo k s p g dw res_mode training dtype act wver fp8_entry stem", defaults=(False,))


def _cba_forward(x, w32, g32, b32, rm, rv, k, s, p, g, act, res, res_mode, training, eps, momentum, cache=None, bn_apply=True, ver=None):
    _require_gpu(x)
    dtype = _COMPUTE_DTYPE
    B, Cin, H, W = x.shape
    dw = g > 1 and g == Cin and g == w32.shape[0]
    qent = None
    if WEIGHT_QUANT and not dw:
        w32, qtok = QUANT.lookup(w32, ver[0] if ver is not None else None)
        qent = QUANT.last
        ver = ((qtok,), (qtok,) + (ver[1] if ver is not None else (g32._version, b32._version, rm._version, rv._version)))
    Cout, Cg_w, kh, kw = w32.shape
    assert kh == k and kw == k and Cin // g == Cg_w, "Conv: weight shape does not match input"
    if Cin == 3 and k == 3 and s == 2 and p == 1 and g == 1 and not x.requires_grad:
        return _stem_forward(x, w32, g32, b32, rm, rv, act, res, res_mode, training, eps, momentum, cache, ver)
    c = ce(dtype)
    if Cin % c != 0:
        if g != 1:
            raise Y3DError(f"grouped conv with {Cin} channels is not 16-byte chunkable")
        Cin_k = (Cin + c - 1) // c * c
        xin = nhwc_empty(B, Cin_k, H, W, dtype, x.device)
        lib().nchw_to_nhwc(code(dtype), x.float().contiguous().data_ptr(), xin.data_ptr(), B, Cin, H, W, Cin_k, stream())
    else:
        xin = to_nhwc(x, dtype)
    if dw:
        return _dw_forward(xin, w32, g32, b32, rm, rv, k, s, p, act, res, res_mode, training, eps, momentum, cache, bn_apply, ver)
    return _dense_forward(xin, w32, g32, b32, rm, rv, Cin, k, s, p, g, act, res, res_mode, training, eps, momentum, cache, bn_apply, ver, qent, True)


def _stem_image(x):
    if x.dtype == torch.uint8:
        hwc = int(not x.is_contiguous() and x.permute(0, 2, 3, 1).is_contiguous())
        return (x if (hwc or x.is_contiguous()) else x.contiguous()), hwc
    return x.float().contiguous(), 0


def _stem_forward(x, w32, g32, b32, rm, rv, act, res, res_mode, training, eps, momentum, cache, ver):
    L, st, dtype, dev = lib(), stream(), _COMPUTE_DTYPE, x.device
    dt = code(dtype)
    B, _, H, W = x.shape
    Cout = w32.shape[0]
    Ho, Wo = (H - 1) // 2 + 1, (W - 1) // 2 + 1
    wkey = ("stemcol", PARAM_EPOCH, w32.data_ptr(), ver[0] if ver is not None else w32._version)
    wcol = cache.get(wkey) if (cache is not None and not training) else None
    if wcol is None:
        wcol = torch.zeros(Cout, 32, dtype=torch.float32, device=dev)
        wcol[:, :27] = w32.detach().permute(0, 2, 3, 1).reshape(Cout, 27)
        if cache is not None and not training:
            _cache_put(cache, wkey, wcol)
    w1x1 = wcol.view(Cout, 32, 1, 1)
    fused = dtype == torch.bfloat16 and Cout % 16 == 0 and 16 <= Cout <= 80 and STEM_FUSED and x.dtype in (torch.uint8, torch.float32)
    if fused and not training and not res_mode:
        _, ss = _eval_consts(cache, "dense", w1x1, g32, b32, rm, rv, ver, dtype, 1, 1, 32, 32, Cout, eps)
        xs, hwc = _stem_image(x)
        mode = 1 + hwc if xs.dtype == torch.uint8 else 0
        ye = out_tensor(B, Cout, Ho, Wo, dtype, dev)
        _timed(("conv_eval", dt, B, H, W, 3, Cout, 3, 2, 1, 1),
               lambda: L.stem_conv_eval(xs.data_ptr(), mode, wcol.data_ptr(), ss[0].data_ptr(), ss[1].data_ptr(), int(act), ye.data_ptr(), ye.stride(3),
                                        B, H, W, Cout, st))
        return ye, None, None
    xcol = nhwc_empty(B, 32, Ho, Wo, dtype, dev)
    xs, hwc = _stem_image(x)
    if fused and training:
        mode = 1 + hwc if xs.dtype == torch.uint8 else 0
        rows = L.stem_conv_train_rows(B, H, W)
        ypre = nhwc_empty(B, Cout, Ho, Wo, dtype, dev)
        part = _f32(rows * Cout * 2, dev)
        _timed(("conv_fwd", dt, B, H, W, 3, Cout, 3, 2, 1),
               lambda: L.stem_conv_train(xs.data_ptr(), mode, wcol.data_ptr(), ypre.data_ptr(), ypre.stride(3), xcol.data_ptr(), part.data_ptr(), B, H, W, Cout, st))
        z, plan, saved = _bn_act_tail(xcol, w1x1, ypre, part, rows, None, g32, b32, rm, rv, 32, 1, 1, 0, 1, act, res, res_mode, training, eps, momentum,
                                      True, None, None)
    else:
        if xs.dtype == torch.uint8:
            L.stem_im2col_u8(dt, xs.data_ptr(), hwc, xcol.data_ptr(), B, H, W, Ho, Wo, st)
        else:
            L.stem_im2col(dt, xs.data_ptr(), xcol.data_ptr(), B, H, W, Ho, Wo, st)
        z, plan, saved = _dense_forward(xcol, w1x1, g32, b32, rm, rv, 32, 1, 1, 0, 1, act, res, res_mode, training, eps, momentum, cache, True, None,
                                        None, False)
    return z, (plan._replace(stem=True) if plan is not None else None), saved


def _dw_forward(xin, w32, g32, b32, rm, rv, k, s, p, act, res, res_mode, training, eps, momentum, cache, bn_apply, ver):
    L, st, dtype, dev = lib(), stream(), xin.dtype, xin.device
    dt = code(dtype)
    B, C, H, W = xin.shape
    Ho, Wo = (H + 2 * p - k) // s + 1, (W + 2 * p - k) // s + 1
    sb, sh, sw = s3(xin)
    fused = not training and bn_apply and DW_EVAL_FUSED
    y = None if fused else nhwc_empty(B, C, Ho, Wo, dtype, dev)
    nblk = L.dw_blocks(B * Ho * Wo)
    part = ss_eval = None
    if training:
        part = _f32(nblk * C * 2, dev)
        wp = _f32(k * k * C, dev)
        L.dw_pack_weight(w32.data_ptr(), wp.data_ptr(), C, k, k, st)
    else:
        wp, ss_eval = _eval_consts(cache, "dw", w32, g32, b32, rm, rv, ver, dtype, k, C, 1, 1, C, eps)
        if fused:
            ze = out_tensor(B, C, Ho, Wo, dtype, dev)
            rr = to_nhwc(res, dtype, dense=True) if res_mode else None
            if rr is not None:
                assert rr.shape == ze.shape, "residual shape mismatch"
            L.dwconv2d_fwd_affine(dt, xin.data_ptr(), sb, sh, sw, B, H, W, C, wp.data_ptr(), ss_eval[0].data_ptr(), ss_eval[1].data_ptr(), int(act),
                                  res_mode, rr.data_ptr() if rr is not None else None, rr.stride(3) if rr is not None else 0,
                                  ze.data_ptr(), ze.stride(3), Ho, Wo, k, k, s, p, st)
            return ze, None, None
    L.dwconv2d_fwd(dt, xin.data_ptr(), sb, sh, sw, B, H, W, C, wp.data_ptr(), y.data_ptr(), C, Ho, Wo, k, k, s, p,
                   part.data_ptr() if training else None, st)
    return _bn_act_tail(xin, w32, y, part, nblk, ss_eval, g32, b32, rm, rv, C, k, s, p, C, act, res, res_mode, training, eps, momentum, bn_apply,
                        ver[0] if ver is not None else None, None)


def _dense_forward(xin, w32, g32, b32, rm, rv, Cin, k, s, p, g, act, res, res_mode, training, eps, momentum, cache, bn_apply, ver, qent, pack_cache):
    L, st, dtype, dev = lib(), stream(), xin.dtype, xin.device
    dt = code(dtype)
    B, Cin_k, H, W = xin.shape
    Cout = w32.shape[0]
    Ho, Wo = (H + 2 * p - k) // s + 1, (W + 2 * p - k) // s + 1
    sb, sh, sw = s3(xin)
    wver = ver[0] if ver is not None else None
    y = nhwc_empty(B, Cout, Ho, Wo, dtype, dev) if (training or res_mode) else None
    f8 = (FP8_CONV and qent is not None and dtype == torch.bfloat16 and k == 3 and s == 1 and p == 1 and Cin_k == Cin
          and bool(L.conv3x3_fp8_ok(B, H, W, Cin, Cout, g)))
    nblk = L.conv3x3_fp8_stat_rows(B, H, W) if f8 else L.conv2d_stat_rows(dt, B, H, W, Cin_k, Cout, g, k, k, s, p)
    part = _f32(nblk * Cout * 2, dev) if training else None
    Cg_pad = Cin_k // g
    wp = ss_eval = None
    if not training:
        wp, ss_eval = _eval_consts(cache, "dense", w32, g32, b32, rm, rv, ver, dtype, k, g, Cin // g, Cg_pad, Cout, eps)
    if f8:
        xq, xs = fp8_input(xin)
        wq, ws = fp8_weight(qent, Cin // g)
        if not training and not res_mode:
            ye = out_tensor(B, Cout, Ho, Wo, dtype, dev)
            _timed(("conv_eval_fp8", dt, B, H, W, Cin_k, Cout, k, s, g, p),
                   lambda: L.conv3x3_fp8_fwd(xq.data_ptr(), xs.data_ptr(), B, H, W, Cin, wq.data_ptr(), ws.data_ptr(), ye.data_ptr(), ye.stride(3), Cout, g, None,
                                             ss_eval[0].data_ptr(), ss_eval[1].data_ptr(), int(act), st))
            return ye, None, None
        _timed(("conv_fwd_fp8", dt, B, H, W, Cin_k, Cout, k, s, g),
               lambda: L.conv3x3_fp8_fwd(xq.data_ptr(), xs.data_ptr(), B, H, W, Cin, wq.data_ptr(), ws.data_ptr(), y.data_ptr(), y.stride(3), Cout, g,
                                         part.data_ptr() if training else None, None, None, 0, st))
    elif not training and not res_mode:
        ye = out_tensor(B, Cout, Ho, Wo, dtype, dev)
        _timed(("conv_eval", dt, B, H, W, Cin_k, Cout, k, s, g, p),
               lambda: L.conv2d_fwd_affine(dt, xin.data_ptr(), sb, sh, sw, B, H, W, Cin_k, wp.data_ptr(), ss_eval[0].data_ptr(), ss_eval[1].data_ptr(),
                                           int(act), ye.data_ptr(), ye.stride(3), Ho, Wo, Cout, g, k, k, s, p, st))
        return ye, None, None
    elif (not training and res_mode == 1 and dtype == torch.bfloat16
            and L.conv2d_fwd_affine_res_ok(dt, B, H, W, Cin_k, Cout, g, k, k, s, p)):
        rr = to_nhwc(res, dtype, dense=True)
        ye = out_tensor(B, Cout, Ho, Wo, dtype, dev)
        L.conv2d_fwd_affine_res(dt, xin.data_ptr(), sb, sh, sw, B, H, W, Cin_k, wp.data_ptr(), ss_eval[0].data_ptr(), ss_eval[1].data_ptr(), int(act),
                                rr.data_ptr(), rr.stride(3), ye.data_ptr(), ye.stride(3), Ho, Wo, Cout, g, k, k, s, p, st)
        return ye, None, None
    else:
        if training and pack_cache and PACK_CACHE:
            wp = PACK_FWD.lookup(w32, w32.data_ptr(), (Cout, Cin // g, Cg_pad, k * k, k * k * Cg_pad, dt), dtype, wver)
        elif training:
            wp = torch.empty(Cout * k * k * Cg_pad, dtype=dtype, device=dev)
            L.pack_weight_fwd(dt, w32.data_ptr(), wp.data_ptr(), Cout, Cin // g, Cg_pad, k, k, st)
        _timed(("conv_fwd", dt, B, H, W, Cin_k, Cout, k, s, g),
               lambda: L.conv2d_fwd(dt, xin.data_ptr(), sb, sh, sw, B, H, W, Cin_k, wp.data_ptr(), None, y.data_ptr(), Cout, Ho, Wo, Cout, g,
                                    k, k, s, p, part.data_ptr() if training else None, st))
    return _bn_act_tail(xin, w32, y, part, nblk, ss_eval, g32, b32, rm, rv, Cin, k, s, p, g, act, res, res_mode, training, eps, momentum, bn_apply,
                        wver, qent if f8 else None)


def _bn_act_tail(xin, w32, y, part, nblk, ss_eval, g32, b32, rm, rv, Cin, k, s, p, g, act, res, res_mode, training, eps, momentum, bn_apply, wver,
                 fp8_entry):
    L, st, dtype, dev = lib(), stream(), y.dtype, y.device
    dt = code(dtype)
    B, Cin_k, H, W = xin.shape
    _, Cout, Ho, Wo = y.shape
    M = B * Ho * Wo
    plan = ConvPlan(B, Cin, Cin_k, H, W, Cout, Ho, Wo, k, s, p, g, g > 1 and g == Cin and g == Cout, res_mode, training, dtype, int(act), wver,
                    fp8_entry)
    if training:
        stats = _f32(6 * Cout, dev).view(6, Cout)
        bump_param_epoch()
        L.bn_finalize(part.data_ptr(), nblk, Cout, M, g32.data_ptr(), b32.data_ptr(), eps, momentum, rm.data_ptr(), rv.data_ptr(),
                      stats[0].data_ptr(), stats[1].data_ptr(), stats[2].data_ptr(), stats[3].data_ptr(), st)
    elif not bn_apply:
        stats = torch.zeros(6, Cout, dtype=torch.float32, device=dev)
        stats[2:4].copy_(ss_eval)
    else:
        stats = None
    if not bn_apply:
        return y, plan, (xin, w32, y, stats, None)
    z = out_tensor(B, Cout, Ho, Wo, dtype, dev)
    rr = None
    if res_mode:
        rr = to_nhwc(res, dtype, dense=True)
        assert rr.shape == z.shape, "residual shape mismatch"
    sc_t, sh_t = (stats[2], stats[3]) if training else (ss_eval[0], ss_eval[1])
    if _FP8_WANT and dtype == torch.bfloat16 and not res_mode and Cout % 64 == 0 and not plan.dw:
        zq = torch.empty(B, Ho, Wo, Cout, dtype=torch.uint8, device=dev)
        zs = torch.empty(B, Ho, Wo, L.fp8_scale_pitch(Cout), dtype=torch.uint8, device=dev)
        L.bn_act_fwd_q(y.data_ptr(), Cout, sc_t.data_ptr(), sh_t.data_ptr(), int(act), z.data_ptr(), z.stride(3), zq.data_ptr(), zs.data_ptr(), M, Cout, st)
        _FP8_ACT[z.data_ptr()] = (zq, zs, (B, Cout, Ho, Wo), z)
    else:
        L.bn_act_fwd(dt, y.data_ptr(), Cout, sc_t.data_ptr(), sh_t.data_ptr(), int(act), res_mode,
                     rr.data_ptr() if rr is not None else None, rr.stride(3) if rr is not None else 0, z.data_ptr(), z.stride(3), M, Cout, st)
    return z, plan, (xin, w32, y, stats, rr if res_mode == 2 else None)


def _cba_backward(plan, saved, dz, need_dx, need_dres, dx_range=None, pre=None, dx_out=None):
    L = lib()
    _, _, y, stats, rr = saved
    B, Cout, Ho, Wo, res_mode, dtype, act = plan.B, plan.Cout, plan.Ho, plan.Wo, plan.res_mode, plan.dtype, plan.act
    if not plan.training:
        raise Y3DError("backward through an eval-mode (running-statistics) Conv is not supported")
    if pre is not None:
        return _conv_backward(plan, saved, pre[0], pre[1], None, need_dx, dx_range, dx_out)
    dt, st, dev = code(dtype), stream(), dz.device
    M = B * Ho * Wo
    dz = to_nhwc(dz, dtype, dense=True)
    nb = L.bn_bwd_blocks(M, Cout)
    part = _f32(nb * Cout * 2, dev)
    rptr = rr.data_ptr() if rr is not None else None
    rsw = rr.stride(3) if rr is not None else 0
    L.bn_act_bwd_reduce(dt, y.data_ptr(), Cout, dz.data_ptr(), dz.stride(3), rptr, rsw, stats[2].data_ptr(), stats[3].data_ptr(),
                        stats[0].data_ptr(), stats[1].data_ptr(), act, res_mode, part.data_ptr(), M, Cout, st)
    dgb = _f32(2 * Cout, dev).view(2, Cout)
    L.bn_bwd_finalize(part.data_ptr(), nb, Cout, M, dgb[0].data_ptr(), dgb[1].data_ptr(), 0, stats[4].data_ptr(), stats[5].data_ptr(), st)
    dy = nhwc_empty(B, Cout, Ho, Wo, dtype, dev)
    dres = None
    if res_mode == 2 and need_dres:
        dres = nhwc_empty(B, Cout, Ho, Wo, dtype, dev)
    L.bn_act_bwd_apply(dt, y.data_ptr(), Cout, dz.data_ptr(), dz.stride(3), rptr, rsw, stats[2].data_ptr(), stats[3].data_ptr(),
                       stats[0].data_ptr(), stats[1].data_ptr(), stats[4].data_ptr(), stats[5].data_ptr(), act, res_mode, 1,
                       dy.data_ptr(), Cout, dres.data_ptr() if dres is not None else None, Cout, M, Cout, st)
    if res_mode == 1:
        dres = dz
    return _conv_backward(plan, saved, dy, dgb, dres, need_dx, dx_range, dx_out)


def _fp8_dgrad_plan(plan, need_dx, dx_range):
    ent = plan.fp8_entry
    if not (FP8_DGRAD and FP8_CONV and need_dx) or ent is None or plan.wver != ((WEIGHT_EPOCH, ent["count"]),):
        return None
    Cin, Cout, g = plan.Cin, plan.Cout, plan.g
    lo, hi = dx_range if dx_range is not None else (0, Cout)
    if plan.Cin_k != Cin or plan.dtype != torch.bfloat16 or (plan.k, plan.s, plan.p) != (3, 1, 1) or (g != 1 and (lo, hi) != (0, Cout)):
        return None
    if (lo, hi) != (0, Cout) and (lo % 128 or (hi - lo) % 128):
        return None
    if not lib().conv3x3_fp8_dgrad_ok(plan.B, plan.H, plan.W, Cin, hi - lo, g):
        return None
    return ent, lo, hi


def _conv_backward(plan, saved, dy, dgb, dres, need_dx, dx_range, dx_out=None):
    L = lib()
    xin, w32 = saved[:2]
    B, Cin, Cin_k, H, W, Cout, Ho, Wo = plan.B, plan.Cin, plan.Cin_k, plan.H, plan.W, plan.Cout, plan.Ho, plan.Wo
    k, s, p, g, dtype = plan.k, plan.s, plan.p, plan.g, plan.dtype
    dt, st = code(dtype), stream()
    dev = dy.device
    esz = 2 if dtype == torch.bfloat16 else 4
    M = B * Ho * Wo
    sb, sh, sw = s3(xin)
    dx = None
    dW = torch.empty_like(w32)
    if plan.dw:
        wp = _f32(k * k * Cout, dev)
        L.dw_pack_weight(w32.data_ptr(), wp.data_ptr(), Cout, k, k, st)
        if need_dx:
            dx = nhwc_empty(B, Cin, H, W, dtype, dev)
            dsb, dsh, dsw = s3(dy)
            L.dwconv2d_bwd_data(dt, dy.data_ptr(), dsb, dsh, dsw, B, Ho, Wo, Cout, wp.data_ptr(), dx.data_ptr(), Cin, H, W, k, k, s, p, st)
        slab = _f32(L.dw_wgrad_blocks(M) * k * k * Cout, dev)
        L.dwconv2d_bwd_weight(dt, xin.data_ptr(), sb, sh, sw, B, H, W, Cin, dy.data_ptr(), Cout, Ho, Wo, k, k, s, p, slab.data_ptr(),
                              dW.data_ptr(), 0, st)
    else:
        f8 = _fp8_dgrad_plan(plan, need_dx, dx_range)
        if f8 is not None and not (px_dense(dy) and dy.data_ptr() % 16 == 0 and dy.stride(3) % 8 == 0):
            f8 = None
        if f8 is not None:
            qent, lo, hi = f8
            wqd, wsd = fp8_weight_dgrad(qent, Cin, g, lo, hi)
            co = hi - lo
            dq = torch.empty(B, Ho, Wo, co, dtype=torch.uint8, device=dev)
            ds = torch.empty(B, Ho, Wo, L.fp8_scale_pitch(co), dtype=torch.uint8, device=dev)
            L.fp8_quantize_grad(dy.data_ptr() + lo * esz, dy.stride(3), qent["scale"].data_ptr() + lo * 4, M, co, dq.data_ptr(), ds.data_ptr(), st)
            dx = dx_out if dx_out is not None else nhwc_empty(B, Cin, H, W, dtype, dev)
            if not (px_dense(dx) and dx.data_ptr() % 16 == 0 and dx.stride(3) % 8 == 0):
                raise Y3DError("fp8 data gradient: dx must be a pixel-dense NHWC tensor with 16-byte aligned rows")
            _timed(("conv_dgrad_fp8", dt, B, H, W, Cin, hi - lo, k, s, g),
                   lambda: L.conv3x3_fp8_dgrad(dq.data_ptr(), ds.data_ptr(), co, ds.shape[3], 0, co, B, H, W, wqd.data_ptr(), wsd.data_ptr(),
                                               dx.data_ptr(), dx.stride(3), Cin, g, st))
        elif need_dx and Cin_k == Cin:
            lo, hi = dx_range if dx_range is not None else (0, Cout)
            assert g == 1 or (lo, hi) == (0, Cout)
            co = hi - lo
            kp = L.conv_kpad(dt, k * k * (co // g))
            src = w32.data_ptr() + lo * (Cin // g) * k * k * 4
            if plan.stem or not PACK_CACHE:
                wpd = torch.empty(Cin * kp, dtype=dtype, device=dev)
                L.pack_weight_dgrad(dt, src, wpd.data_ptr(), co, Cin // g, g, k, k, st)
            else:
                wpd = PACK_DGRAD.lookup(w32, src, (g, co // g, Cin // g, k * k, kp, dt), dtype, plan.wver)
            dx = dx_out if dx_out is not None else nhwc_empty(B, Cin, H, W, dtype, dev)
            dsb, dsh, dsw = s3(dy)
            _timed(("conv_dgrad", dt, B, H, W, Cin, co, k, s, g),
                   lambda: L.conv2d_bwd_data(dt, dy.data_ptr() + lo * esz, dsb, dsh, dsw, B, Ho, Wo, co, wpd.data_ptr(), dx.data_ptr(), dx.stride(3), H, W,
                                             Cin, g, k, k, s, p, st))
        ns = L.conv2d_wgrad_plan(dt, B, H, W, Cin_k, Cout, g, k, k, s, p)
        slab = _f32(ns * Cout * k * k * (Cin_k // g), dev)
        _timed(("conv_wgrad", dt, B, H, W, Cin_k, Cout, k, s, g),
               lambda: L.conv2d_bwd_weight(dt, xin.data_ptr(), sb, sh, sw, B, H, W, Cin_k, Cin, dy.data_ptr(), Cout, Ho, Wo, Cout, g, k, k,
                                           s, p, slab.data_ptr(), ns, dW.data_ptr(), 0, st))
    if plan.stem:
        dW = dW.reshape(Cout, 32)[:, :27].reshape(Cout, 3, 3, 3).permute(0, 3, 1, 2).contiguous()
        dx = None
    return dx, dW, dgb[0], dgb[1], dres


def _w32(weight):
    w = weight.detach()
    if w.dtype != torch.float32 or not w.is_contiguous():
        w = w.float().contiguous()
    return w


class ConvBNActFn(torch.autograd.Function):

    @staticmethod
    def forward(ctx, x, weight, gamma, beta, res, res_mode, m):
        z, cfg, saved = _cba_forward(x, _w32(weight), gamma.detach().float(), beta.detach().float(), m.bn.running_mean, m.bn.running_var,
                                     m.k, m.s, m.p, m.g, m.has_act, res, res_mode, m.training, m.eps, m.momentum,
                                     m.__dict__.setdefault("_eval_cache", {}))
        if m.training:
            m._nbt_pending += 1
        ctx.cfg = cfg
        if saved is not None:
            ctx.save_for_backward(*saved)
        return z

    @staticmethod
    def backward(ctx, dz):
        if ctx.cfg is None:
            raise Y3DError("backward through an eval-mode (running-statistics) Conv is not supported")
        dx, dW, dg, db, dres = _cba_backward(ctx.cfg, ctx.saved_tensors, dz, ctx.needs_input_grad[0], ctx.needs_input_grad[4])
        return dx, dW, dg, db, dres, None, None


class StackedConvs:

    def __init__(self, convs, groups=1):
        self.convs = list(convs)
        self.groups = groups
        self.couts = [c.conv.out_channels for c in self.convs]
        self.flat = {}

    def _ensure(self, name, tensors, setter):
        flat = self.flat.get(name)
        ok = flat is not None and flat.device == tensors[0].device
        if ok:
            base, off = flat.data_ptr(), 0
            for t in tensors:
                if t.data_ptr() != base + off * 4:
                    ok = False
                    break
                off += t.numel()
        if not ok:
            flat = torch.cat([t.detach().reshape(-1).float() for t in tensors])
            off = 0
            for i, t in enumerate(tensors):
                n = t.numel()
                setter(i, flat[off:off + n].view(t.shape))
                off += n
            self.flat[name] = flat
        return flat

    def tensors(self):
        cs = self.convs
        w = self._ensure("w", [c.conv.weight for c in cs], lambda i, v: setattr(cs[i].conv.weight, "data", v))
        gm = self._ensure("g", [c.bn.weight for c in cs], lambda i, v: setattr(cs[i].bn.weight, "data", v))
        bt = self._ensure("b", [c.bn.bias for c in cs], lambda i, v: setattr(cs[i].bn.bias, "data", v))
        rm = self._ensure("rm", [c.bn.running_mean for c in cs], lambda i, v: cs[i].bn._buffers.__setitem__("running_mean", v))
        rv = self._ensure("rv", [c.bn.running_var for c in cs], lambda i, v: cs[i].bn._buffers.__setitem__("running_var", v))
        c0 = cs[0].conv
        wv = tuple(c.conv.weight._version for c in cs)
        self.ver = (wv, wv + tuple(t._version for c in cs for t in (c.bn.weight, c.bn.bias, c.bn.running_mean, c.bn.running_var)))
        return w.view(sum(self.couts), c0.in_channels // c0.groups, *c0.kernel_size), gm, bt, rm, rv

    def params(self):
        return [c.conv.weight for c in self.convs] + [c.bn.weight for c in self.convs] + [c.bn.bias for c in self.convs]


class FusedConvBNActFn(torch.autograd.Function):

    @staticmethod
    def forward(ctx, x, stack, groups, dx_range, *params):
        w, gm, bt, rm, rv = stack.tensors()
        m = stack.convs[0]
        z, cfg, saved = _cba_forward(x, w, gm, bt, rm, rv, m.k, m.s, m.p, groups, m.has_act, None, 0, m.training, m.eps, m.momentum, ver=stack.ver)
        if m.training:
            for c in stack.convs:
                c._nbt_pending += 1
        ctx.cfg, ctx.couts, ctx.dx_range = cfg, stack.couts, dx_range
        ctx.gslot = grad_slot(x) if (m.training and torch.is_tensor(x) and x.is_cuda) else None
        if saved is not None:
            ctx.save_for_backward(*saved)
        return z

    @staticmethod
    def backward(ctx, dz):
        dx_out = grad_slot_tensor(ctx.gslot) if (ctx.gslot is not None and ctx.needs_input_grad[0]) else None
        dx, dW, dg, db, _ = _cba_backward(ctx.cfg, ctx.saved_tensors, dz, ctx.needs_input_grad[0], False, ctx.dx_range, dx_out=dx_out)
        dWs, dgs, dbs, off = [], [], [], 0
        for co in ctx.couts:
            dWs.append(dW[off:off + co])
            dgs.append(dg[off:off + co])
            dbs.append(db[off:off + co])
            off += co
        return (dx, None, None, None, *dWs, *dgs, *dbs)


# ... 552 lines not shown
```

Measured before the change: 1458.

## Rework wgrad slab fold, tile weight packing through LDS, cache depthwise packed weights

Adds a row-oriented wgrad reduction kernel that sums float4 slab chunks and stages the result in LDS, so the OIHW gradient is written with coalesced vector stores instead of scattered scalar stores. The split is chosen by a memoized cost heuristic. It also rewrites the multi-tensor weight pack kernel to transpose through a larger LDS tile with vectorized stores. Depthwise packed weights now go through the pack cache instead of being repacked on every call, and the projection slab reduction is unrolled. The extra LDS footprint may lower occupancy, and the larger kernel surface adds correctness risk.

```diff
diff --git a/include/y3d.h b/include/y3d.h
--- a/include/y3d.h
+++ b/include/y3d.h
@@ -74,6 +74,8 @@
 int y3d_conv2d_bwd_weight(int dtype, const void* x, int64_t xsb, int64_t xsh, int64_t xsw, int B, int H, int W, int Cin,
                           int Cin_real, const void* dy, int64_t dsw, int Ho, int Wo, int Cout, int groups, int kh, int kw,
                           int stride, int pad, float* slab, int nsplit, float* grad_oihw, int accumulate, void* stream);
+int y3d_wgrad_fold(const float* slab, int nsplit, int Cout, int taps, int Cin_g, int Cin_g_real, float* grad_oihw, int accumulate,
+                   void* stream);
 
 int y3d_dw_blocks(int64_t M);
 int y3d_dw_wgrad_blocks(int64_t M);
@@ -90,6 +92,7 @@
 int y3d_dwconv2d_bwd_weight(int dtype, const void* x, int64_t xsb, int64_t xsh, int64_t xsw, int B, int H, int W, int C,
                             const void* dy, int64_t dsw, int Ho, int Wo, int kh, int kw, int stride, int pad, float* slab,
                             float* grad_oihw, int accumulate, void* stream);
+int y3d_dw_wgrad_fold(const float* slab, int nblk, int C, int taps, float* grad_oihw, int accumulate, void* stream);
 
 int y3d_bn_finalize(const float* partials, int nblk, int C, int64_t count, const float* gamma, const float* beta, float eps,
                     float momentum, float* running_mean, float* running_var, float* mean, float* invstd, float* scale,
diff --git a/yolov10-3d_amd/csrc/common.h b/yolov10-3d_amd/csrc/common.h
--- a/yolov10-3d_amd/csrc/common.h
+++ b/yolov10-3d_amd/csrc/common.h
@@ -86,6 +86,23 @@
   return v;
 }
 
+__device__ __forceinline__ void store_image_f32(const float* img, float* out, int cnt, int accumulate) {
+  const int mis = (int)(((uintptr_t)out >> 2) & 3);
+  for (int k = threadIdx.x; 4 * k < cnt + mis; k += 256) {
+    const int lo = 4 * k - mis;
+    if (lo >= 0 && lo + 4 <= cnt) {
+      float4 v = make_float4(img[lo], img[lo + 1], img[lo + 2], img[lo + 3]);
+      float4* o = (float4*)(out + lo);
+      if (accumulate) { const float4 a = *o; v.x = a.x + v.x; v.y = a.y + v.y; v.z = a.z + v.z; v.w = a.w + v.w; }
+      *o = v;
+    } else {
+#pragma unroll
+      for (int j = 0; j < 4; ++j)
+        if (lo + j >= 0 && lo + j < cnt) out[lo + j] = accumulate ? out[lo + j] + img[lo + j] : img[lo + j];
+    }
+  }
+}
+
 void y3d_set_error(const char* fmt, ...);
 #define Y3D_CHECK(cond, ...)          \
   do {                                \
diff --git a/yolov10-3d_amd/csrc/conv_gemm.hip b/yolov10-3d_amd/csrc/conv_gemm.hip
--- a/yolov10-3d_amd/csrc/conv_gemm.hip
+++ b/yolov10-3d_amd/csrc/conv_gemm.hip
@@ -505,50 +505,114 @@
   }
 }
 
+constexpr int FOLD_CAP = 6144;
+
 template <int SL>
-__global__ __launch_bounds__(256) void wgrad_reduce_scalar_kernel(const float* __restrict__ slab, float* __restrict__ grad, int nsplit, int Ctot,
-                                                           int taps, int Cg, int Cg_real, int accumulate) {
-  constexpr int EPB = 256 / SL;
-  __shared__ float sh[SL][EPB];
-  const int e = threadIdx.x % EPB, sl = threadIdx.x / EPB;
-  long idx = (long)blockIdx.x * EPB + e;
-  long n = (long)Ctot * taps * Cg;
-  float s = 0.f;
-  if (idx < n) {
-    float s0 = 0.f, s1 = 0.f, s2 = 0.f, s3 = 0.f;
-    int k = sl;
-    for (; k + 3 * SL < nsplit; k += 4 * SL) {
-      s0 += slab[(long)k * n + idx];
-      s1 += slab[(long)(k + SL) * n + idx];
-      s2 += slab[(long)(k + 2 * SL) * n + idx];
-      s3 += slab[(long)(k + 3 * SL) * n + idx];
-    }
-    for (; k < nsplit; k += SL) s0 += slab[(long)k * n + idx];
-    s = (s0 + s1) + (s2 + s3);
-  }
-  if (SL > 1) {
-    sh[sl][e] = s;
-    __syncthreads();
-    if (sl != 0) return;
-#pragma unroll
-    for (int j = 1; j < SL; ++j) s += sh[j][e];
-  }
-  if (idx >= n) return;
-  int ci = idx % Cg;
-  int tap = (idx / Cg) % taps;
-  int co = idx / ((long)Cg * taps);
-  if (ci >= Cg_real) return;
-  long o = ((long)co * Cg_real + ci) * taps + tap;
-  grad[o] = accumulate ? grad[o] + s : s;
-}
-
-inline void launch_wgrad_reduce(const float* slab, float* grad, int nsplit, int Ctot, int taps, int Cg, int Cg_real, int accumulate, hipStream_t st) {
-  long n = (long)Ctot * taps * Cg;
-  long ng = (n + 3) / 4;
-  if (n <= 65536 && nsplit >= 64) hipLaunchKernelGGL(wgrad_reduce_kernel<16>, dim3(cdiv(ng, 16)), dim3(256), 0, st, slab, grad, nsplit, Ctot, taps, Cg, Cg_real, accumulate);
-  else if (n <= 1048576 && nsplit >= 32) hipLaunchKernelGGL(wgrad_reduce_kernel<8>, dim3(cdiv(ng, 32)), dim3(256), 0, st, slab, grad, nsplit, Ctot, taps, Cg, Cg_real, accumulate);
-  else if (nsplit >= 8) hipLaunchKernelGGL(wgrad_reduce_kernel<2>, dim3(cdiv(ng, 128)), dim3(256), 0, st, slab, grad, nsplit, Ctot, taps, Cg, Cg_real, accumulate);
-  else hipLaunchKernelGGL(wgrad_reduce_scalar_kernel<1>, dim3(cdiv(n, 256)), dim3(256), 0, st, slab, grad, nsplit, Ctot, taps, Cg, Cg_real, accumulate);
+__global__ __launch_bounds__(256) void wgrad_reduce_rows_kernel(const float* __restrict__ slab, float* __restrict__ grad, int nsplit, int Ctot,
+                                                                int taps, int Cg, int Cg_real, int accumulate, int R, int CC) {
+  constexpr int GPB = 256 / SL;
+  __shared__ float4 sh[SL > 1 ? 2 * 256 : 1];
+  __shared__ __attribute__((aligned(16))) float img[FOLD_CAP];
+  const int e = threadIdx.x % GPB, sl = threadIdx.x / GPB;
+  const int nch = (Cg + CC - 1) / CC;
+  int co0, c0, rows;
+  if (nch == 1) {
+    co0 = blockIdx.x * R; c0 = 0; rows = Ctot - co0 < R ? Ctot - co0 : R;
+  } else {
+    co0 = blockIdx.x / nch; c0 = (blockIdx.x - co0 * nch) * CC; rows = 1;
+  }
+  const int cc = Cg - c0 < CC ? Cg - c0 : CC;
+  const int q = cc >> 2, per = taps * q, ng = rows * per;
+  const long n = (long)Ctot * taps * Cg;
+  int par = 0;
+  for (int g0 = 0; g0 < ng; g0 += GPB, par ^= 1) {
+    const int g = g0 + e;
+    int r = 0, tap = 0, c4 = 0;
+    float4 s = make_float4(0.f, 0.f, 0.f, 0.f);
+    if (g < ng) {
+      r = g / per;
+      const int rem = g - r * per;
+      tap = rem / q;
+      c4 = rem - tap * q;
+      const float* src = slab + ((long)(co0 + r) * taps + tap) * Cg + c0 + 4 * c4;
+      float4 s0 = s, s1 = s, s2 = s, s3 = s;
+      auto add = [](float4& a, const float4 b) { a.x += b.x; a.y += b.y; a.z += b.z; a.w += b.w; };
+      int k = sl;
+      for (; k + 3 * SL < nsplit; k += 4 * SL) {
+        const float4 v0 = *(const float4*)(src + (long)k * n), v1 = *(const float4*)(src + (long)(k + SL) * n);
+        const float4 v2 = *(const float4*)(src + (long)(k + 2 * SL) * n), v3 = *(const float4*)(src + (long)(k + 3 * SL) * n);
+        add(s0, v0); add(s1, v1); add(s2, v2); add(s3, v3);
+      }
+      for (; k < nsplit; k += SL) add(s0, *(const float4*)(src + (long)k * n));
+      s.x = (s0.x + s1.x) + (s2.x + s3.x); s.y = (s0.y + s1.y) + (s2.y + s3.y);
+      s.z = (s0.z + s1.z) + (s2.z + s3.z); s.w = (s0.w + s1.w) + (s2.w + s3.w);
+    }
+    if (SL > 1) {
+      sh[(par * SL + sl) * GPB + e] = s;
+      __syncthreads();
+      if (sl == 0) {
+#pragma unroll
+        for (int j = 1; j < SL; ++j) { const float4 v = sh[(par * SL + j) * GPB + e]; s.x += v.x; s.y += v.y; s.z += v.z; s.w += v.w; }
+      }
+    }
+    if (sl == 0 && g < ng) {
+      const float v[4] = {s.x, s.y, s.z, s.w};
+      float* d = img + ((long)r * Cg_real + 4 * c4) * taps + tap;
+#pragma unroll
+      for (int j = 0; j < 4; ++j)
+        if (c0 + 4 * c4 + j < Cg_real) d[j * taps] = v[j];
+    }
+  }
+  __syncthreads();
+  int creal = Cg_real - c0 < cc ? Cg_real - c0 : cc;
+  if (creal < 0) creal = 0;
+  store_image_f32(img, grad + ((long)co0 * Cg_real + c0) * taps, rows * creal * taps, accumulate);
+}
+
+struct FoldShape { int Ctot, taps, Cg, GPB, R, CC, grid; };
+
+inline FoldShape wgrad_fold_shape(int Ctot, int taps, int Cg, int GPB) {
+  constexpr int NMEMO = 64;
+  thread_local FoldShape memo[NMEMO];
+  thread_local int nmemo = 0;
+  for (int i = 0; i < (nmemo < NMEMO ? nmemo : NMEMO); ++i)
+    if (memo[i].Ctot == Ctot && memo[i].taps == taps && memo[i].Cg == Cg && memo[i].GPB == GPB) return memo[i];
+  FoldShape f = {Ctot, taps, Cg, GPB, 0, 0, 0};
+  const int q = Cg / 4;
+  long best = -1;
+  int bestG = 0;
+  auto consider = [&](int r, int cc, long blocks, int G) {
+    const long cost = (long)cdiv(blocks, 1024) * cdiv(G, GPB);
+    if (best < 0 || cost < best || (cost == best && G > bestG)) { best = cost; bestG = G; f.R = r; f.CC = cc; f.grid = (int)blocks; }
+  };
+  for (int qq = 16; qq < q && 4L * qq * taps <= FOLD_CAP; ++qq) consider(1, 4 * qq, (long)Ctot * cdiv(q, qq), taps * qq);
+  for (int r = 1; r <= Ctot && (long)r * Cg * taps <= FOLD_CAP; ++r) consider(r, Cg, cdiv(Ctot, r), r * taps * q);
+  memo[nmemo++ % NMEMO] = f;
+  return f;
+}
+
+inline int launch_wgrad_reduce(const float* slab, float* grad, int nsplit, int Ctot, int taps, int Cg, int Cg_real, int accumulate, hipStream_t st) {
+  Y3D_CHECK(Cg % 4 == 0 && ((uintptr_t)slab & 15) == 0, "wgrad fold: the slabs are read as 16-byte chunks of four input channels");
+  const long n = (long)Ctot * taps * Cg;
+  const long ng = n / 4;
+  if (n <= 65536 && nsplit >= 64) {
+    hipLaunchKernelGGL(wgrad_reduce_kernel<16>, dim3(cdiv(ng, 16)), dim3(256), 0, st, slab, grad, nsplit, Ctot, taps, Cg, Cg_real, accumulate);
+  } else if (n <= 1048576 && nsplit >= 32) {
+    hipLaunchKernelGGL(wgrad_reduce_kernel<8>, dim3(cdiv(ng, 32)), dim3(256), 0, st, slab, grad, nsplit, Ctot, taps, Cg, Cg_real, accumulate);
+  } else {
+    const int SL = nsplit >= 8 ? 2 : 1;
+    const FoldShape f = wgrad_fold_shape(Ctot, taps, Cg, 256 / SL);
+    if (f.grid == 0) {
+      if (SL == 2) hipLaunchKernelGGL(wgrad_reduce_kernel<2>, dim3(cdiv(ng, 128)), dim3(256), 0, st, slab, grad, nsplit, Ctot, taps, Cg, Cg_real, accumulate);
+      else hipLaunchKernelGGL(wgrad_reduce_kernel<1>, dim3(cdiv(ng, 256)), dim3(256), 0, st, slab, grad, nsplit, Ctot, taps, Cg, Cg_real, accumulate);
+    } else if (SL == 2) {
+      hipLaunchKernelGGL(wgrad_reduce_rows_kernel<2>, dim3(f.grid), dim3(256), 0, st, slab, grad, nsplit, Ctot, taps, Cg, Cg_real, accumulate, f.R, f.CC);
+    } else {
+      hipLaunchKernelGGL(wgrad_reduce_rows_kernel<1>, dim3(f.grid), dim3(256), 0, st, slab, grad, nsplit, Ctot, taps, Cg, Cg_real, accumulate, f.R, f.CC);
+    }
+  }
+  Y3D_LAUNCH_CHECK();
+  return Y3D_OK;
 }
 
 template <typename T>
@@ -582,62 +646,179 @@
   TT<T>::st(out + idx, v);
 }
 
+constexpr int PACK_CAP = 8192;
+
+template <typename OT>
+__device__ __forceinline__ void pack_store_linear(const float* img, OT* __restrict__ out, int count, bool vec, int tid) {
+  constexpr int E = TT<OT>::CE;
+  if (vec) {
+    for (int p = tid * E; p < count; p += 256 * E) {
+      float f[E];
+#pragma unroll
+      for (int j = 0; j < E; j += 4) {
+        const float4 v = *(const float4*)(img + p + j);
+        f[j] = v.x; f[j + 1] = v.y; f[j + 2] = v.z; f[j + 3] = v.w;
+      }
+      *(uint4*)(out + p) = Chunk<OT>::pack(f);
+    }
+  } else {
+    for (int i = tid; i < count; i += 256) TT<OT>::st(out + i, img[i]);
+  }
+}
+
+template <typename OT>
+__device__ __forceinline__ void pack_cols_pass(const float* __restrict__ w, OT* __restrict__ out, float* img, int b, int c, int taps, int Kpad,
+                                               int g, int ci0, long r0, int nr, int co0, int cb, int P, bool vec, int tid) {
+  constexpr int E = TT<OT>::CE;
+  const int seg = nr * taps;
+  const long cs = (long)c * taps;
+  const float* __restrict__ base = w + ((long)(g * b + co0) * c + ci0) * taps;
+  if (((uintptr_t)w & 15) == 0 && seg % 4 == 0 && cs % 4 == 0 && ((long)ci0 * taps) % 4 == 0) {
+    const int sq = seg >> 2;
+    for (int i = tid; i < cb * sq; i += 256) {
+      const int col = i / sq, j = 4 * (i - col * sq);
+      const float4 v = *(const float4*)(base + col * cs + j);
+      float* d = img + j * P + col;
+      d[0] = v.x; d[P] = v.y; d[2 * P] = v.z; d[3 * P] = v.w;
+    }
+  } else {
+    for (int i = tid; i < cb * seg; i += 256) {
+      const int col = i / seg, j = i - col * seg;
+      img[j * P + col] = base[col * cs + j];
+    }
+  }
+  __syncthreads();
+  if (vec) {
+    const int pc = cb / E;
+    for (int p = tid; p < seg * pc; p += 256) {
+      const int j = p / pc, col = (p - j * pc) * E;
+      const int cil = j / taps, tap = j - cil * taps;
+      float f[E];
+#pragma unroll
+      for (int jj = 0; jj < E; ++jj) f[jj] = img[j * P + col + jj];
+      *(uint4*)(out + (r0 + cil) * Kpad + (long)tap * b + co0 + col) = Chunk<OT>::pack(f);
+    }
+  } else {
+    for (int o = tid; o < seg * cb; o += 256) {
+      const int j = o / cb, col = o - j * cb;
+      const int cil = j / taps, tap = j - cil * taps;
+      TT<OT>::st(out + (r0 + cil) * Kpad + (long)tap * b + co0 + col, img[j * P + col]);
+    }
+  }
+}
+
+template <typename OT>
+__device__ __forceinline__ void pack_cols(const float* __restrict__ w, OT* __restrict__ out, float* img, int b, int c, int taps, int Kpad, long rb,
+                                          long re, int tid) {
+  constexpr int E = TT<OT>::CE;
+  bool vec = ((uintptr_t)out & 15) == 0 && b % E == 0 && Kpad == taps * b;
+  int CB = b < 128 ? b : 128;
+  if ((long)taps * (CB | 1) > PACK_CAP) CB = PACK_CAP / taps - 1;
+  if (vec && CB >= E) CB -= CB % E;
+  else vec = false;
+  const int P = CB | 1;
+  int R = PACK_CAP / (taps * P);
+  if (R >= 4) R &= ~3;
+  for (long r0 = rb; r0 < re;) {
+    const int g = (int)(r0 / c), ci0 = (int)(r0 - (long)g * c);
+    int nr = R;
+    if (nr > c - ci0) nr = c - ci0;
+    if (nr > re - r0) nr = (int)(re - r0);
+    const int over = (ci0 + nr) & 3;
+    if (over && nr > over && ci0 + nr < c) nr -= over;
+    for (int co0 = 0; co0 < b; co0 += CB) {
+      __syncthreads();
+      pack_cols_pass<OT>(w, out, img, b, c, taps, Kpad, g, ci0, r0, nr, co0, b - co0 < CB ? b - co0 : CB, P, vec, tid);
+    }
+    if (Kpad != taps * b) {
+      const int np = Kpad - taps * b;
+      for (int o = tid; o < nr * np; o += 256) {
+        const int rl = o / np;
+        TT<OT>::st(out + (r0 + rl) * Kpad + taps * b + (o - rl * np), 0.f);
+      }
+    }
+    r0 += nr;
+  }
+}
+
 template <typename T>
 __global__ __launch_bounds__(256) void mt_pack_w_kernel(const long* __restrict__ desc, const int* __restrict__ ctensor, const int* __restrict__ coff,
                                                         int chunk) {
-  constexpr int CAP = 4096;
-  __shared__ float st[CAP + 64];
+  constexpr int E = TT<T>::CE;
+  __shared__ __attribute__((aligned(16))) float img[PACK_CAP];
   const long* d = desc + (long)ctensor[blockIdx.x] * 8;
   const float* __restrict__ w = (const float*)d[0];
-  T* __restrict__ out = (T*)d[1];
   const int a = (int)d[2], b = (int)d[3], c = (int)d[4], taps = (int)d[5], Kpad = (int)d[6], mode = (int)d[7];
   const long n = mode == 0 ? (long)a * Kpad : (long)a * c * Kpad;
   const long beg = (long)coff[blockIdx.x] * chunk;
   const long end = beg + chunk < n ? beg + chunk : n;
   const int tid = threadIdx.x;
-  const long rb = beg / Kpad, re = (end - 1) / Kpad;
-  if (mode == 0) {
-    for (long idx = beg + tid; idx < end; idx += 256) {
-      const int k = (int)(idx % Kpad), co = (int)(idx / Kpad);
+  const long rb = (beg + Kpad - 1) / Kpad, re = (end + Kpad - 1) / Kpad;
+  if (rb >= re) return;
+  if ((mode == 0 && Kpad > PACK_CAP) || taps > PACK_CAP / 2) {
+    for (long idx = rb * Kpad + tid; idx < re * Kpad; idx += 256) {
+      const int k = (int)(idx % Kpad);
+      const long row = idx / Kpad;
       float v = 0.f;
-      if (k < taps * c) {
-        const int tap = k / c, ci = k - tap * c;
-        if (ci < b) v = w[((long)co * b + ci) * taps + tap];
-      }
-      TT<T>::st(out + idx, v);
-    }
+      if (mode == 0) {
+        if (k < taps * c) {
+          const int tap = k / c, ci = k - tap * c;
+          if (ci < b) v = w[(row * b + ci) * taps + tap];
+        }
+      } else if (k < taps * b) {
+        const int tap = k / b, co = k - tap * b;
+        const long g = row / c, ci = row - g * c;
+        v = w[((g * b + co) * c + ci) * taps + tap];
+      }
+      if (mode == 2) ((float*)d[1])[idx] = v;
+      else TT<T>::st((T*)d[1] + idx, v);
+    }
+    return;
+  }
+  if (mode == 2) {
+    pack_cols<float>(w, (float*)d[1], img, b, c, taps, Kpad, rb, re, tid);
+  } else if (mode == 1) {
+    pack_cols<T>(w, (T*)d[1], img, b, c, taps, Kpad, rb, re, tid);
   } else {
-    const int CB = b < 256 ? b : 256;
-    int R = CAP / (taps * (CB + 1));
-    if (R < 1) R = 1;
-    const int P = CB + 1;
-    for (long r0 = rb; r0 <= re;) {
-      const int g = (int)(r0 / c), ci0 = (int)(r0 - (long)g * c);
-      int nr = R;
-      if (nr > c - ci0) nr = c - ci0;
-      if (nr > re - r0 + 1) nr = (int)(re - r0 + 1);
-      const int seg = nr * taps;
-      for (int co0 = 0; co0 < b; co0 += CB) {
-        const int cb = b - co0 < CB ? b - co0 : CB;
+    T* __restrict__ out = (T*)d[1];
+    const bool vec = ((uintptr_t)out & 15) == 0 && Kpad % E == 0;
+    const bool pad = c != b || Kpad != taps * c;
+    const int RP = PACK_CAP / Kpad, L = b * taps;
+    const bool quad = ((uintptr_t)w & 15) == 0 && L % 4 == 0;
+    for (long r0 = rb; r0 < re; r0 += RP) {
+      const int nr = re - r0 < RP ? (int)(re - r0) : RP;
+      const int tot = nr * L;
+      const float* __restrict__ src = w + r0 * L;
+      __syncthreads();
+      if (pad) {
+        for (int i = tid; i < nr * Kpad; i += 256) img[i] = 0.f;
         __syncthreads();
-        for (int i = tid; i < cb * seg; i += 256) {
-          const int col = i / seg, j = i - col * seg;
-          st[j * P + col] = w[((long)(g * b + co0 + col) * c + ci0) * taps + j];
+      }
+      if (quad && taps == 1 && !pad) {
+        for (int i = 4 * tid; i < tot; i += 1024) *(float4*)(img + i) = *(const float4*)(src + i);
+      } else if (quad) {
+        for (int i = 4 * tid; i < tot; i += 1024) {
+          const float4 v = *(const float4*)(src + i);
+          const float vv[4] = {v.x, v.y, v.z, v.w};
+          const int rc = i / taps;
+          int tap = i - rc * taps, rl = rc / b, ci = rc - rl * b;
+#pragma unroll
+          for (int j = 0; j < 4; ++j) {
+            img[rl * Kpad + tap * c + ci] = vv[j];
+            if (++tap == taps) {
+              tap = 0;
+              if (++ci == b) { ci = 0; ++rl; }
+            }
+          }
         }
-        __syncthreads();
-        for (int o = tid; o < seg * cb; o += 256) {
-          const int j = o / cb, col = o - j * cb;
-          const int cil = j / taps, tap = j - cil * taps;
-          const long idx = (r0 + cil) * Kpad + (long)tap * b + co0 + col;
-          if (idx >= beg && idx < end) TT<T>::st(out + idx, st[j * P + col]);
+      } else {
+        for (int i = tid; i < tot; i += 256) {
+          const int rc = i / taps, tap = i - rc * taps, rl = rc / b, ci = rc - rl * b;
+          img[rl * Kpad + tap * c + ci] = src[i];
         }
       }
-      for (int o = tid; o < nr * (Kpad - taps * b); o += 256) {
-        const int rl = o / (Kpad - taps * b), k = taps * b + o - rl * (Kpad - taps * b);
-        const long idx = (r0 + rl) * Kpad + k;
-        if (idx >= beg && idx < end) TT<T>::st(out + idx, 0.f);
-      }
-      r0 += nr;
+      __syncthreads();
+      pack_store_linear<T>(img, out + r0 * Kpad, nr * Kpad, vec, tid);
     }
   }
 }
@@ -1000,25 +1181,19 @@
   if (route == Y3D_ROUTE_WGRAD_SMALL) {
     int rc = y3d_wgrad3x3_small_launch(x, xsb, xsh, xsw, dy, dsw, B, H, W, Cin, Cout, slab, nsplit, stream);
     if (rc) return rc;
-    launch_wgrad_reduce(slab, grad_oihw, nsplit, Cout, 9, Cin, Cin, accumulate, st);
-    Y3D_LAUNCH_CHECK();
-    return Y3D_OK;
+    return launch_wgrad_reduce(slab, grad_oihw, nsplit, Cout, 9, Cin, Cin, accumulate, st);
   }
   if (route == Y3D_ROUTE_WGRAD_TILE) {
     const int th = y3d_wgrad_tile_height(dtype, H, W, p.Cg, p.Cn, kh, kw, stride, pad);
     Y3D_CHECK(nsplit == y3d_wgrad_tile_splits(th, B, H, W, p.Cg, p.Cn, groups), "conv2d_bwd_weight: nsplit must come from y3d_conv2d_wgrad_plan");
     int rc = y3d_conv3x3_wgrad_tile_launch(th, x, xsb, xsh, xsw, dy, dsw, B, H, W, p.Cg, p.Cn, groups, slab, nsplit, stream);
     if (rc) return rc;
-    launch_wgrad_reduce(slab, grad_oihw, nsplit, Cout, kh * kw, p.Cg, p.Cg, accumulate, st);
-    Y3D_LAUNCH_CHECK();
-    return Y3D_OK;
+    return launch_wgrad_reduce(slab, grad_oihw, nsplit, Cout, kh * kw, p.Cg, p.Cg, accumulate, st);
   }
   if (route == Y3D_ROUTE_WGRAD_STREAM1X1) {
     int rc = y3d_wgrad1x1_stream_launch(x, xsw, dy, dsw, p.M, Cin, Cout, slab, nsplit, p.chunk_px, stream);
     if (rc) return rc;
-    launch_wgrad_reduce(slab, grad_oihw, nsplit, Cout, 1, Cin, Cin, accumulate, st);
-    Y3D_LAUNCH_CHECK();
-    return Y3D_OK;
+    return launch_wgrad_reduce(slab, grad_oihw, nsplit, Cout, 1, Cin, Cin, accumulate, st);
   }
   const int wd = wgrad_tile_w(p.Cn), wx = wgrad_tile_w(p.Ktot);
   dim3 grid(cdiv(p.Ktot, wx), cdiv(p.Cn, wd), groups * nsplit);
@@ -1036,9 +1211,12 @@
 #undef Y3D_WGRAD
   Y3D_LAUNCH_CHECK();
   int cg_real = groups == 1 ? Cin_real : p.Cg;
-  launch_wgrad_reduce(slab, grad_oihw, nsplit, Cout, kh * kw, p.Cg, cg_real, accumulate, st);
-  Y3D_LAUNCH_CHECK();
-  return Y3D_OK;
+  return launch_wgrad_reduce(slab, grad_oihw, nsplit, Cout, kh * kw, p.Cg, cg_real, accumulate, st);
+}
+
+int y3d_wgrad_fold(const float* slab, int nsplit, int Cout, int taps, int Cin_g, int Cin_g_real, float* grad_oihw, int accumulate, void* stream) {
+  Y3D_CHECK(slab && grad_oihw && nsplit >= 1 && Cout >= 1 && Cin_g_real >= 1 && Cin_g_real <= Cin_g, "wgrad_fold: bad argument");
+  return launch_wgrad_reduce(slab, grad_oihw, nsplit, Cout, taps, Cin_g, Cin_g_real, accumulate, (hipStream_t)stream);
 }
 
 int y3d_mt_pack_weights(int dtype, const int64_t* desc, const int* chunk_tensor, const int* chunk_off, int nchunks, int chunk, void* stream) {
diff --git a/yolov10-3d_amd/csrc/dwconv.hip b/yolov10-3d_amd/csrc/dwconv.hip
--- a/yolov10-3d_amd/csrc/dwconv.hip
+++ b/yolov10-3d_amd/csrc/dwconv.hip
@@ -332,6 +332,12 @@
     else if (dgrad) { if (kk == 3) DW_LAUNCH_K(T, true, 3); else if (kk == 7) DW_LAUNCH_K(T, true, 7); else DW_LAUNCH_K(T, true, 0); }     \
     else { if (kk == 3) DW_LAUNCH_K(T, false, 3); else if (kk == 7) DW_LAUNCH_K(T, false, 7); else DW_LAUNCH_K(T, false, 0); }        \
   } while (0)
+
+static int dw_launch_fold(const float* slab, float* grad, int nblk, int taps, int C, int accumulate, hipStream_t st) {
+  hipLaunchKernelGGL(dw_wgrad_reduce_kernel, dim3(cdiv((long)C * taps, 32)), dim3(256), 0, st, slab, grad, nblk, taps, C, accumulate);
+  Y3D_LAUNCH_CHECK();
+  return Y3D_OK;
+}
 
 static int dw_launch(int dtype, bool dgrad, const DwP& p, hipStream_t st) {
   Y3D_CHECK(p.M < (1L << 31), "dwconv: more than 2^31 pixels");
@@ -433,9 +439,12 @@
   if (dtype == Y3D_BF16) Y3D_DWW(bf16_t); else Y3D_DWW(float);
 #undef Y3D_DWW
   Y3D_LAUNCH_CHECK();
-  hipLaunchKernelGGL(dw_wgrad_reduce_kernel, dim3(cdiv((long)C * kh * kw, 32)), dim3(256), 0, st, slab, grad_oihw, nblk, kh * kw, C, accumulate);
-  Y3D_LAUNCH_CHECK();
-  return Y3D_OK;
-}
-
-}
+  return dw_launch_fold(slab, grad_oihw, nblk, kh * kw, C, accumulate, st);
+}
+
+int y3d_dw_wgrad_fold(const float* slab, int nblk, int C, int taps, float* grad_oihw, int accumulate, void* stream) {
+  Y3D_CHECK(slab && grad_oihw && nblk >= 1 && C >= 1 && taps >= 1, "dw_wgrad_fold: bad argument");
+  return dw_launch_fold(slab, grad_oihw, nblk, taps, C, accumulate, (hipStream_t)stream);
+}
+
+}
diff --git a/yolov10-3d_amd/csrc/proj_bn_mfma.hip b/yolov10-3d_amd/csrc/proj_bn_mfma.hip
--- a/yolov10-3d_amd/csrc/proj_bn_mfma.hip
+++ b/yolov10-3d_amd/csrc/proj_bn_mfma.hip
@@ -306,19 +306,25 @@
   if (tid < cout) p.bslab[(long)blockIdx.x * p.ctot + p.ooff[br] + tid] = bred[0][tid] + bred[1][tid] + bred[2][tid] + bred[3][tid];
 }
 
+__device__ __forceinline__ float slab_sum_in_order(const float* __restrict__ src, long pitch, int nblk) {
+  float s = 0.f;
+  int b = 0;
+  for (; b + 8 <= nblk; b += 8) {
+    float v[8];
+#pragma unroll
+    for (int j = 0; j < 8; ++j) v[j] = src[(long)(b + j) * pitch];
+#pragma unroll
+    for (int j = 0; j < 8; ++j) s += v[j];
+  }
+  for (; b < nblk; ++b) s += src[(long)b * pitch];
+  return s;
+}
+
 __global__ void projg_wslab_reduce_kernel(PWP p, int nblk, int cin) {
   const int br = blockIdx.y, cout = p.cout[br];
   const int idx = blockIdx.x * blockDim.x + threadIdx.x;
-  if (idx < cout * cin) {
-    float s = 0.f;
-    for (int b = 0; b < nblk; ++b) s += p.slab[((long)b * p.ctot + p.ooff[br]) * cin + idx];
-    p.dw[br][idx] = s;
-  }
-  if (idx < cout) {
-    float s = 0.f;
-    for (int b = 0; b < nblk; ++b) s += p.bslab[(long)b * p.ctot + p.ooff[br] + idx];
-    p.db[br][idx] = s;
-  }
+  if (idx < cout * cin) p.dw[br][idx] = slab_sum_in_order(p.slab + (long)p.ooff[br] * cin + idx, (long)p.ctot * cin, nblk);
+  if (idx < cout) p.db[br][idx] = slab_sum_in_order(p.bslab + p.ooff[br] + idx, p.ctot, nblk);
 }
 
 }
diff --git a/yolov10-3d_amd/ops.py b/yolov10-3d_amd/ops.py
--- a/yolov10-3d_amd/ops.py
+++ b/yolov10-3d_amd/ops.py
@@ -252,6 +252,8 @@
 
 class _PackRegistry(_WeightRegistry):
 
+    DW = 2
+
     CHUNK = 16384
 
     def __init__(self, mode):
@@ -262,7 +264,9 @@
         L, st = lib(), stream()
         a, b, c, taps, kpad, dt = e["geo"]
         k = int(round(taps ** 0.5))
-        if self.mode == 0:
+        if e["mode"] == self.DW:
+            L.dw_pack_weight(e["src"], e["dst"].data_ptr(), b, k, k, st)
+        elif e["mode"] == 0:
             L.pack_weight_fwd(dt, e["src"], e["dst"].data_ptr(), a, b, c, k, k, st)
         else:
             L.pack_weight_dgrad(dt, e["src"], e["dst"].data_ptr(), a * b, c, a, k, k, st)
@@ -277,8 +281,8 @@
             desc, ct, co = [], [], []
             for t, e in enumerate(ents):
                 a, b, c, taps, kpad, _ = e["geo"]
-                n = a * kpad if self.mode == 0 else a * c * kpad
-                desc += [e["src"], e["dst"].data_ptr(), a, b, c, taps, kpad, self.mode]
+                n = a * kpad if e["mode"] == 0 else a * c * kpad
+                desc += [e["src"], e["dst"].data_ptr(), a, b, c, taps, kpad, e["mode"]]
                 for j in range((n + self.CHUNK - 1) // self.CHUNK):
                     ct.append(t)
                     co.append(j)
@@ -289,15 +293,16 @@
         lib().mt_pack_weights(dt, desc.data_ptr(), ct.data_ptr(), co.data_ptr(), n, self.CHUNK, stream())
         return ents
 
-    def lookup(self, w32, src_ptr, geo, dtype, ver=None):
-        key = (src_ptr, geo)
+    def lookup(self, w32, src_ptr, geo, dtype, ver=None, mode=None):
+        mode = self.mode if mode is None else mode
+        key = (src_ptr, geo, mode)
         ver = w32._version if ver is None else ver
         e = self.entries.get(key)
         if e is None:
             a, b, c, taps, kpad, dt = geo
-            n = a * kpad if self.mode == 0 else a * c * kpad
-            e = {"src": src_ptr, "geo": geo, "dst": torch.empty(n, dtype=dtype, device=w32.device), "ver": ver, "seen": WEIGHT_EPOCH,
-                 "keep": w32}
+            n = a * kpad if mode == 0 else a * c * kpad
+            e = {"src": src_ptr, "geo": geo, "mode": mode, "dst": torch.empty(n, dtype=dtype, device=w32.device), "ver": ver,
+                 "seen": WEIGHT_EPOCH, "keep": w32}
             self.entries[key] = e
             self._pack_one(e)
         elif self._revisit(e, (WEIGHT_EPOCH, geo[5]), ver, lambda: self._pack_all(geo[5])):
@@ -348,6 +353,16 @@
 
 
 PACK_FWD, PACK_DGRAD, QUANT = _PackRegistry(0), _PackRegistry(1), _QuantRegistry()
+
+
+def _dw_packed(w32, C, k, dtype, ver):
+    if PACK_CACHE:
+        return PACK_FWD.lookup(w32, w32.data_ptr(), (1, C, 1, k * k, k * k * C, code(dtype)), torch.float32, ver, _PackRegistry.DW)
+    wp = _f32(k * k * C, w32.device)
+    lib().dw_pack_weight(w32.data_ptr(), wp.data_ptr(), C, k, k, stream())
+    return wp
+
+
 WEIGHT_QUANT = None
 
 
@@ -605,8 +620,7 @@
     part = ss_eval = None
     if training:
         part = _f32(nblk * C * 2, dev)
-        wp = _f32(k * k * C, dev)
-        L.dw_pack_weight(w32.data_ptr(), wp.data_ptr(), C, k, k, st)
+        wp = _dw_packed(w32, C, k, dtype, ver[0] if ver is not None else None)
     else:
         wp, ss_eval = _eval_consts(cache, "dw", w32, g32, b32, rm, rv, ver, dtype, k, C, 1, 1, C, eps)
         if fused:
@@ -776,8 +790,7 @@
     dx = None
     dW = torch.empty_like(w32)
     if plan.dw:
-        wp = _f32(k * k * Cout, dev)
-        L.dw_pack_weight(w32.data_ptr(), wp.data_ptr(), Cout, k, k, st)
+        wp = _dw_packed(w32, Cout, k, dtype, plan.wver)
         if need_dx:
             dx = nhwc_empty(B, Cin, H, W, dtype, dev)
             dsb, dsh, dsw = s3(dy)
```

After: 1477 (median of 6 runs). 1.2% higher.
